# Gregor-Mendel-Institute/SNPmatch

Measured on NVIDIA B200. Metric: snp_accession_comparisons_per_sec, higher is better.
Workload: dtype f64

## Files before the change

### snpmatch_b200/csrc/api.cu

```cuda
#include "common.cuh"
#include <atomic>
#include <memory>
#include <new>
#include "pack.cuh"
#include "join.cuh"
#include "score.cuh"
#include "windows.cuh"
#include "f1.cuh"
#include "hardcall.cuh"
#include "gemm_onehot.cuh"
#include "grouped.cuh"
#include "group_sort.cuh"
#include "grouped2.cuh"
#include "pairs.cuh"
#include "pair_matrix.cuh"
#include "cross_geno.cuh"
#include <unordered_map>

namespace snpm {
thread_local std::string g_last_error;

static int grid_for(int64_t items, int threads, int n_sm, int per_sm = 16) {
    int64_t g = ceil_div64(items, threads);
    const int64_t cap = int64_t(n_sm) * per_sm;
// ... 558 lines not shown
        } else {
            SNPM_CUDA(cudaMemcpyAsync(b->d_wei.p, wei, size_t(n) * 24, cudaMemcpyHostToDevice, st));
        }
    }
    SNPM_CUDA(cudaEventRecord(b->ev_uploaded, st));
    b->ran = b->ran_windows = b->epilogue_done = false;
    return SNPM_OK;
}

static int batch_new(snpm_db *db, snpm_batch **out) {
    snpm_batch *b = new snpm_batch();
    b->db = db;
    for (int i = 0; i < SNPM_N_EVENTS; ++i) {
        if (cudaEventCreate(&b->ev[i]) != cudaSuccess) { snpm_batch_destroy(b); return fail(SNPM_E_CUDA, "cudaEventCreate failed"); }
    }
    if (cudaStreamCreateWithFlags(&b->copy_stream, cudaStreamNonBlocking) != cudaSuccess ||
        cudaEventCreateWithFlags(&b->ev_uploaded, cudaEventDisableTiming) != cudaSuccess ||
        cudaEventCreateWithFlags(&b->ev_inputs_free, cudaEventDisableTiming) != cudaSuccess ||
        cudaEventCreate(&b->ev_joined) != cudaSuccess) {
        snpm_batch_destroy(b);
        return fail(SNPM_E_CUDA, "snpm_batch_create: copy stream / events");
    }
    if (cudaMallocHost(reinterpret_cast<void **>(&b->h_status), 8 * sizeof(int)) != cudaSuccess) {
        snpm_batch_destroy(b);
        return fail(SNPM_E_NOMEM, "cudaMallocHost failed");
    }
    *out = b;
    return SNPM_OK;
}

int snpm_batch_create(snpm_db *db, int64_t n_samples, const int64_t *offsets, const int32_t *s_chrom_id, const int32_t *s_pos,
                      const double *wei, snpm_batch **out) {
    if (!db || !out) return fail(SNPM_E_ARG, "snpm_batch_create: NULL handle");
    *out = nullptr;
    SNPM_CUDA(cudaSetDevice(db->device));
    snpm_batch *b = nullptr;
    SNPM_TRY(batch_new(db, &b));
    int rc = batch_upload(b, n_samples, offsets, s_chrom_id, s_pos, wei);
    if (rc == SNPM_OK && cudaStreamSynchronize(b->copy_stream) != cudaSuccess) rc = fail(SNPM_E_CUDA, "snpm_batch_create: upload failed");
    if (rc != SNPM_OK) { snpm_batch_destroy(b); return rc; }
    *out = b;
    return SNPM_OK;
}

int snpm_batch_upload(snpm_batch *b, int64_t n_samples, const int64_t *offsets, const int32_t *s_chrom_id, const int32_t *s_pos,
                      const double *wei) {
    if (!b) return fail(SNPM_E_ARG, "snpm_batch_upload: NULL batch");
    SNPM_CUDA(cudaSetDevice(b->db->device));
    return batch_upload(b, n_samples, offsets, s_chrom_id, s_pos, wei);
}

int snpm_batch_upload_indexed(snpm_batch *b, int64_t n_samples, const int64_t *offsets, const int32_t *s_chrom_id, const int32_t *s_pos,
                              const uint16_t *wei_idx, const double *table, int32_t n_table) {
    if (!b) return fail(SNPM_E_ARG, "snpm_batch_upload_indexed: NULL batch");
    if (!wei_idx && offsets && n_samples >= 1 && offsets[n_samples] > 0) return fail(SNPM_E_ARG, "snpm_batch_upload_indexed: NULL weight indices");
    SNPM_CUDA(cudaSetDevice(b->db->device));
    return batch_upload(b, n_samples, offsets, s_chrom_id, s_pos, nullptr, wei_idx, table, n_table);
}


int snpm_group_markers(int64_t n_samples, const int64_t *offsets, const int32_t *s_chrom_id, const int32_t *s_pos, const double *wei,
                       uint8_t *out_chrom, int32_t *out_pos, uint16_t *out_gid, int64_t *out_order, double *table, int32_t table_cap,
                       int32_t *n_table) {
    if (n_samples < 1 || !offsets || !n_table || !table || table_cap < 1) return fail(SNPM_E_ARG, "snpm_group_markers: bad arguments");
    const int64_t n = offsets[n_samples];
    if (n > 0 && (!s_chrom_id || !s_pos || !wei || !out_chrom || !out_pos || !out_gid)) return fail(SNPM_E_ARG, "snpm_group_markers: NULL marker arrays");
    struct Key {
        uint64_t a, b, c;
        bool operator==(const Key &o) const { return a == o.a && b == o.b && c == o.c; }
    };
    struct KeyHash {
        size_t operator()(const Key &k) const {
            uint64_t h = k.a * 0x9E3779B97F4A7C15ull;
            h ^= (k.b + 0x7F4A7C15ull) * 0xC2B2AE3D27D4EB4Full + (h << 6) + (h >> 2);
            h ^= (k.c + 0x165667B19E3779F9ull) * 0xFF51AFD7ED558CCDull + (h << 6) + (h >> 2);
            return size_t(h ^ (h >> 29));
        }
    };
    std::unordered_map<Key, int32_t, KeyHash> ids;
    ids.reserve(4096);
    const int32_t cap = std::min<int32_t>(table_cap, 65536);
    std::vector<int32_t> gid(static_cast<size_t>(n));
    for (int64_t i = 0; i < n; ++i) {
        const double w0 = wei[3 * i], w1 = wei[3 * i + 1], w2 = wei[3 * i + 2];
        if (!(w0 >= 0.0 && w1 >= 0.0 && w2 >= 0.0) || std::isinf(w0) || std::isinf(w1) || std::isinf(w2))
            return fail(SNPM_E_ARG, "snpm_group_markers: weights must be finite and non-negative (marker %lld)", (long long)i);
        Key k;
        memcpy(&k.a, &w0, 8);
        memcpy(&k.b, &w1, 8);
        memcpy(&k.c, &w2, 8);
        if (w0 == 0.0) k.a = 0;
        if (w1 == 0.0) k.b = 0;
        if (w2 == 0.0) k.c = 0;
        auto it = ids.find(k);
        if (it == ids.end()) {
            const int32_t id = int32_t(ids.size());
            if (id >= cap) return fail(SNPM_E_RANGE, "snpm_group_markers: more than %d distinct weight triples", cap);
            table[3 * size_t(id)] = w0;
            table[3 * size_t(id) + 1] = w1;
            table[3 * size_t(id) + 2] = w2;
            it = ids.emplace(k, id).first;
        }
        gid[size_t(i)] = it->second;
        const int32_t c = s_chrom_id[i];
        if (c >= 255) return fail(SNPM_E_RANGE, "snpm_group_markers: chromosome id %d does not fit one byte", c);
    }
    const int32_t T = int32_t(ids.size());
    *n_table = T;
    {
        std::vector<int32_t> called(static_cast<size_t>(T));
        std::vector<std::vector<double>> seen(9);
        for (int32_t t = 0; t < T; ++t) {
            const double *w = table + 3 * size_t(t);
            int c = 0;
            if (w[0] == 1.0) c = 0; else if (w[2] == 1.0) c = 2; else if (w[1] == 1.0) c = 1;
            else { c = 0; if (w[2] > w[c]) c = 2; if (w[1] > w[c]) c = 1; }
            called[size_t(t)] = c;
            for (int k = 0; k < 3; ++k) seen[size_t(3 * c + k)].push_back(w[k]);
        }
        int slow[3], fast[3];
        for (int c = 0; c < 3; ++c) {
            size_t distinct[3] = {0, 0, 0};
            for (int k = 0; k < 3; ++k) {
                auto &v = seen[size_t(3 * c + k)];
                std::sort(v.begin(), v.end());
                distinct[k] = size_t(std::unique(v.begin(), v.end()) - v.begin());
            }
            const int o1 = (c + 1) % 3, o2 = (c + 2) % 3;
            if (distinct[o1] <= distinct[o2]) { slow[c] = o1; fast[c] = o2; } else { slow[c] = o2; fast[c] = o1; }
        }
        std::vector<int32_t> perm(static_cast<size_t>(T)), rank(static_cast<size_t>(T));
        for (int32_t t = 0; t < T; ++t) perm[size_t(t)] = t;
        std::sort(perm.begin(), perm.end(), [&](int32_t x, int32_t y) {
            const int cx = called[size_t(x)], cy = called[size_t(y)];
            if (cx != cy) return cx < cy;
            const double *wx_ = table + 3 * size_t(x), *wy_ = table + 3 * size_t(y);
            if (wx_[cx] != wy_[cx]) return wx_[cx] > wy_[cx];
            if (wx_[slow[cx]] != wy_[slow[cx]]) return wx_[slow[cx]] > wy_[slow[cx]];
            if (wx_[fast[cx]] != wy_[fast[cx]]) return wx_[fast[cx]] > wy_[fast[cx]];
            return x < y;
        });
        std::vector<double> sorted(static_cast<size_t>(T) * 3);
        for (int32_t r = 0; r < T; ++r) {
            rank[size_t(perm[size_t(r)])] = r;
            memcpy(&sorted[3 * size_t(r)], table + 3 * size_t(perm[size_t(r)]), 24);
        }
        memcpy(table, sorted.data(), size_t(T) * 24);
        for (int64_t i = 0; i < n; ++i) gid[size_t(i)] = rank[size_t(gid[size_t(i)])];
    }
    std::vector<int64_t> cnt(static_cast<size_t>(T) + 1);
    for (int64_t s = 0; s < n_samples; ++s) {
        const int64_t b0 = offsets[s], b1 = offsets[s + 1];
        std::fill(cnt.begin(), cnt.end(), 0);
        for (int64_t i = b0; i < b1; ++i) ++cnt[size_t(gid[size_t(i)]) + 1];
        for (int32_t t = 0; t < T; ++t) cnt[size_t(t) + 1] += cnt[size_t(t)];
        for (int64_t i = b0; i < b1; ++i) {
            const int32_t g = gid[size_t(i)];
            const int64_t o = b0 + cnt[size_t(g)]++;
            out_chrom[o] = s_chrom_id[i] < 0 ? uint8_t(255) : uint8_t(s_chrom_id[i]);
            out_pos[o] = s_pos[i];
            out_gid[o] = uint16_t(g);
            if (out_order) out_order[o] = i;
        }
    }
    return SNPM_OK;
}

static int upload_grouped(snpm_batch *b, int64_t n_samples, const int64_t *offsets, const uint8_t *chrom_u8, const int32_t *s_pos,
                          const uint32_t *packed_cp, const uint16_t *gid, const double *table, int32_t n_table,
                          const uint16_t *run_gid = nullptr, const uint32_t *run_end = nullptr, int64_t n_runs = 0) {
    if (!b) return fail(SNPM_E_ARG, "snpm_batch_upload_grouped: NULL batch");
    snpm_db *db = b->db;
    if (n_samples < 1 || !offsets || offsets[0] != 0) return fail(SNPM_E_ARG, "snpm_batch_upload_grouped: need samples and offsets starting at 0");
    for (int64_t s = 0; s < n_samples; ++s)
        if (offsets[s + 1] < offsets[s]) return fail(SNPM_E_ARG, "snpm_batch_upload_grouped: offsets must be non-decreasing");
    const int64_t n = offsets[n_samples];
    if (n >= (int64_t(1) << 31) - 2048) return fail(SNPM_E_ARG, "snpm_batch_upload_grouped: %lld markers exceed the 2^31 limit", (long long)n);
    if (n > 0 && ((!gid && !run_gid) || (!packed_cp && (!chrom_u8 || !s_pos)))) return fail(SNPM_E_ARG, "snpm_batch_upload_grouped: NULL marker arrays");
    if (run_gid && n > 0) {
        if (!run_end || n_runs < 1 || n_runs > n) return fail(SNPM_E_ARG, "snpm_batch_upload_grouped_runs: need 1..n runs");
        if (int64_t(run_end[n_runs - 1]) != n || run_end[0] == 0) return fail(SNPM_E_ARG, "snpm_batch_upload_grouped_runs: the runs must cover markers 0..n");
    }
    if (!table || n_table < 1 || n_table > 65536) return fail(SNPM_E_ARG, "snpm_batch_upload_grouped: weight table must hold 1..65536 triples");
    std::vector<double> t4(size_t(n_table) * 4);
    for (int32_t t = 0; t < n_table; ++t) {
        const double w0 = table[3 * size_t(t)], w1 = table[3 * size_t(t) + 1], w2 = table[3 * size_t(t) + 2];
        if (!(w0 >= 0.0 && w1 >= 0.0 && w2 >= 0.0) || std::isinf(w0) || std::isinf(w1) || std::isinf(w2))
            return fail(SNPM_E_ARG, "snpm_batch_upload_grouped: weights must be finite and non-negative (triple %d)", t);
        t4[4 * size_t(t)] = w0;
        t4[4 * size_t(t) + 1] = w2;
        t4[4 * size_t(t) + 2] = w1;
        t4[4 * size_t(t) + 3] = 0.0;
    }
    SNPM_CUDA(cudaSetDevice(db->device));
    b->S = n_samples;
    b->n = n;
    b->grouped = true;
    b->coded = false;
    b->pending_expand = 0;
    b->n_gtable = n_table;
    b->gchunk = b->gchunk_req;
    b->h_off.assign(offsets, offsets + n_samples + 1);
    int64_t nseg = 0;
    for (int64_t s = 0; s < n_samples; ++s) nseg += ceil_div64(offsets[s + 1] - offsets[s], b->gchunk);
    b->nseg_cap = nseg;
    SNPM_TRY(b->d_off.ensure(size_t(n_samples + 1) * 8));
    SNPM_TRY(b->d_chrom8.ensure(size_t(n)));
    SNPM_TRY(b->d_chrom.ensure(size_t(n) * 4));
    SNPM_TRY(b->d_pos.ensure(size_t(n) * 4));
    SNPM_TRY(b->d_gid.ensure(size_t(n) * 2));
    SNPM_TRY(b->d_gtable.ensure(size_t(n_table) * 32));
    cudaStream_t st = b->copy_stream;
    SNPM_CUDA(cudaStreamWaitEvent(st, b->ev_inputs_free, 0));
    SNPM_CUDA(cudaMemcpyAsync(b->d_off.p, offsets, size_t(n_samples + 1) * 8, cudaMemcpyHostToDevice, st));
    b->h_gtable.assign(t4.begin(), t4.end());
    SNPM_CUDA(cudaMemcpyAsync(b->d_gtable.p, b->h_gtable.data(), size_t(n_table) * 32, cudaMemcpyHostToDevice, st));
    if (n) {
        if (run_gid) {
            const size_t bad_off = (size_t(n_runs) * 6 + 15) & ~size_t(15);
            SNPM_TRY(b->d_runs.ensure(bad_off + 16));
            uint32_t *d_end = b->d_runs.as<uint32_t>();
            uint16_t *d_rg = reinterpret_cast<uint16_t *>(d_end + n_runs);
            b->d_runs_bad = reinterpret_cast<int *>(static_cast<char *>(b->d_runs.p) + bad_off);
            SNPM_CUDA(cudaMemsetAsync(b->d_runs_bad, 0, sizeof(int), st));
            SNPM_CUDA(cudaMemcpyAsync(d_end, run_end, size_t(n_runs) * 4, cudaMemcpyHostToDevice, st));
            SNPM_CUDA(cudaMemcpyAsync(d_rg, run_gid, size_t(n_runs) * 2, cudaMemcpyHostToDevice, st));
            b->pending_expand |= 1;
            b->pending_runs = n_runs;
        } else {
            b->d_runs_bad = nullptr;
            SNPM_CUDA(cudaMemcpyAsync(b->d_gid.p, gid, size_t(n) * 2, cudaMemcpyHostToDevice, st));
        }
        if (packed_cp) {
            SNPM_TRY(b->d_wei_idx.ensure(size_t(n) * 4));
            SNPM_CUDA(cudaMemcpyAsync(b->d_wei_idx.p, packed_cp, size_t(n) * 4, cudaMemcpyHostToDevice, st));
            b->pending_expand |= 2;
        } else {
            SNPM_CUDA(cudaMemcpyAsync(b->d_chrom8.p, chrom_u8, size_t(n), cudaMemcpyHostToDevice, st));
            SNPM_CUDA(cudaMemcpyAsync(b->d_pos.p, s_pos, size_t(n) * 4, cudaMemcpyHostToDevice, st));
            b->pending_expand |= 4;
        }
    }
    SNPM_CUDA(cudaEventRecord(b->ev_uploaded, st));
    b->ran = b->ran_windows = b->epilogue_done = false;
    return SNPM_OK;
}

int snpm_batch_upload_grouped(snpm_batch *b, int64_t n_samples, const int64_t *offsets, const uint8_t *chrom_u8, const int32_t *s_pos,
                              const uint16_t *gid, const double *table, int32_t n_table) {
    return upload_grouped(b, n_samples, offsets, chrom_u8, s_pos, nullptr, gid, table, n_table);
}

int snpm_batch_upload_grouped_packed(snpm_batch *b, int64_t n_samples, const int64_t *offsets, const uint32_t *chrom_pos, const uint16_t *gid,
                                     const double *table, int32_t n_table) {
    return upload_grouped(b, n_samples, offsets, nullptr, nullptr, chrom_pos, gid, table, n_table);
}

int snpm_batch_upload_grouped_runs(snpm_batch *b, int64_t n_samples, const int64_t *offsets, const uint32_t *chrom_pos, const uint16_t *run_gid,
                                   const uint32_t *run_end, int64_t n_runs, const double *table, int32_t n_table) {
    return upload_grouped(b, n_samples, offsets, nullptr, nullptr, chrom_pos, nullptr, table, n_table, run_gid, run_end, n_runs);
}

static int upload_coded(snpm_batch *b, int64_t n_samples, const int64_t *offsets, const uint32_t *chrom_pos, const uint16_t *codes,
                        const uint32_t *codes32, const double *wtable, int32_t n_wtable) {
    if (!b) return fail(SNPM_E_ARG, "snpm_batch_upload_coded: NULL batch");
    if (codes32 && n_wtable > 1024) return fail(SNPM_E_ARG, "snpm_batch_upload_coded32: three codes share one word only up to 1024 weight values (%d given)", n_wtable);
    snpm_db *db = b->db;
    if (n_samples < 1 || !offsets || offsets[0] != 0) return fail(SNPM_E_ARG, "snpm_batch_upload_coded: need samples and offsets starting at 0");
    for (int64_t s = 0; s < n_samples; ++s)
        if (offsets[s + 1] < offsets[s]) return fail(SNPM_E_ARG, "snpm_batch_upload_coded: offsets must be non-decreasing");
    const int64_t n = offsets[n_samples];
    if (n >= (int64_t(1) << 31) - 2048) return fail(SNPM_E_ARG, "snpm_batch_upload_coded: %lld markers exceed the 2^31 limit", (long long)n);
    if (n > 0 && (!chrom_pos || (!codes && !codes32))) return fail(SNPM_E_ARG, "snpm_batch_upload_coded: NULL marker arrays");
    if (!wtable || n_wtable < 1 || n_wtable > 65536) return fail(SNPM_E_ARG, "snpm_batch_upload_coded: the weight table must hold 1..65536 values");
    for (int32_t t = 0; t < n_wtable; ++t)
        if (!(wtable[t] >= 0.0) || std::isinf(wtable[t])) return fail(SNPM_E_ARG, "snpm_batch_upload_coded: weights must be finite and non-negative (entry %d)", t);
    if (!b->gchunk_set) b->gchunk_req = db->stride > G2_WX ? G2_MAX_CHUNK : 320;
    if (b->gchunk_req % GR_BLOCK || b->gchunk_req > G2_MAX_CHUNK)
        return fail(SNPM_E_ARG, "snpm_batch_upload_coded: the group chunk must be a multiple of %d and at most %d rows (it is %d)", GR_BLOCK, G2_MAX_CHUNK, b->gchunk_req);
    SNPM_CUDA(cudaSetDevice(db->device));
    b->S = n_samples;
    b->n = n;
    b->grouped = true;
    b->coded = true;
    b->codes_packed = codes32 != nullptr;
    b->pending_expand = 2;
    b->d_runs_bad = nullptr;
    b->n_wtable = n_wtable;
    int bits = 1;
    while ((1 << bits) < n_wtable) ++bits;
    b->code_bits = bits;
    b->key_bits = 3 * bits + 2;
    b->gchunk = b->gchunk_req;
    b->h_off.assign(offsets, offsets + n_samples + 1);
    int64_t nseg = 0;
    std::vector<int32_t> tile_first(size_t(n_samples) + 1), tile_sample;
    for (int64_t s = 0; s < n_samples; ++s) {
        const int64_t ns = offsets[s + 1] - offsets[s];
        nseg += ceil_div64(ns, b->gchunk);
        tile_first[size_t(s)] = int32_t(tile_sample.size());
        for (int64_t t = 0; t < ceil_div64(ns, RS_TILE); ++t) tile_sample.push_back(int32_t(s));
    }
    tile_first[size_t(n_samples)] = int32_t(tile_sample.size());
    b->nseg_cap = nseg;
    b->n_sort_tiles = int64_t(tile_sample.size());
    const size_t key_bytes = b->key_bits <= 32 ? 4 : 8;
    SNPM_TRY(b->d_off.ensure(size_t(n_samples + 1) * 8));
    SNPM_TRY(b->d_chrom.ensure(size_t(n) * 4));
    SNPM_TRY(b->d_pos.ensure(size_t(n) * 4));
    SNPM_TRY(b->d_wei_idx.ensure(size_t(n) * 4));
    SNPM_TRY(b->d_codes.ensure(size_t(n) * 6));
    SNPM_TRY(b->d_wtable.ensure(size_t(n_wtable) * 8));
    SNPM_TRY(b->d_key_a.ensure(size_t(n) * key_bytes));
    SNPM_TRY(b->d_pair_db_tmp.ensure(size_t(n) * 4));
    SNPM_TRY(b->d_pair_s_tmp.ensure(size_t(n) * 4));
    SNPM_TRY(b->d_tile_sample.ensure(std::max<size_t>(tile_sample.size(), 1) * 4));
    SNPM_TRY(b->d_tile_first.ensure(size_t(n_samples + 1) * 4));
    SNPM_TRY(b->d_tile_hist.ensure(std::max<size_t>(tile_sample.size(), 1) * (size_t(GH_MAX_GROUPS) * 4 + 8)));
    SNPM_TRY(b->d_blk_chg.ensure(size_t(std::max<int64_t>(nseg, 1)) * (size_t(b->gchunk / GR_BLOCK) * 8 + 12) + size_t(SO_BUCKETS) * 4 + 16));
    SNPM_TRY(b->d_seg_order.ensure(size_t(std::max<int64_t>(nseg, 1)) * 16));
    SNPM_TRY(b->d_work_counter.ensure(256));
    SNPM_TRY(b->d_hash.ensure(size_t(n_samples) * GH_SLOTS * 8));
    SNPM_TRY(b->d_slot_gid.ensure(size_t(n_samples) * GH_SLOTS * 2));
    SNPM_TRY(b->d_ngroups.ensure(size_t(n_samples) * 4));
    SNPM_TRY(b->d_group_overflow.ensure(size_t(n_samples) * 4));
    SNPM_TRY(b->d_gkeys.ensure(size_t(n_samples) * GH_MAX_GROUPS * key_bytes));
    SNPM_TRY(b->d_gw.ensure(size_t(n_samples) * GH_MAX_GROUPS * 32));
    SNPM_TRY(b->d_goff.ensure(size_t(n_samples) * (GH_MAX_GROUPS + 1) * 4));
    SNPM_TRY(b->d_gid.ensure(size_t(n) * 2));
    cudaStream_t st = b->copy_stream;
    SNPM_CUDA(cudaStreamWaitEvent(st, b->ev_inputs_free, 0));
    b->h_gtable.assign(wtable, wtable + n_wtable);
    b->h_tiles.assign(tile_first.begin(), tile_first.end());
    b->h_tiles.insert(b->h_tiles.end(), tile_sample.begin(), tile_sample.end());
    SNPM_CUDA(cudaMemcpyAsync(b->d_off.p, offsets, size_t(n_samples + 1) * 8, cudaMemcpyHostToDevice, st));
    SNPM_CUDA(cudaMemcpyAsync(b->d_wtable.p, b->h_gtable.data(), size_t(n_wtable) * 8, cudaMemcpyHostToDevice, st));
    SNPM_CUDA(cudaMemcpyAsync(b->d_tile_first.p, b->h_tiles.data(), size_t(n_samples + 1) * 4, cudaMemcpyHostToDevice, st));
    if (!tile_sample.empty())
        SNPM_CUDA(cudaMemcpyAsync(b->d_tile_sample.p, b->h_tiles.data() + n_samples + 1, tile_sample.size() * 4, cudaMemcpyHostToDevice, st));
    if (n) {
        SNPM_CUDA(cudaMemcpyAsync(b->d_wei_idx.p, chrom_pos, size_t(n) * 4, cudaMemcpyHostToDevice, st));
        if (codes32) SNPM_CUDA(cudaMemcpyAsync(b->d_codes.p, codes32, size_t(n) * 4, cudaMemcpyHostToDevice, st));
        else SNPM_CUDA(cudaMemcpyAsync(b->d_codes.p, codes, size_t(n) * 6, cudaMemcpyHostToDevice, st));
    }
    SNPM_CUDA(cudaEventRecord(b->ev_uploaded, st));
    b->ran = b->ran_windows = b->epilogue_done = false;
    return SNPM_OK;
}

int snpm_batch_upload_coded(snpm_batch *b, int64_t n_samples, const int64_t *offsets, const uint32_t *chrom_pos, const uint16_t *codes,
                            const double *wtable, int32_t n_wtable) {
    return upload_coded(b, n_samples, offsets, chrom_pos, codes, nullptr, wtable, n_wtable);
}

int snpm_batch_upload_coded32(snpm_batch *b, int64_t n_samples, const int64_t *offsets, const uint32_t *chrom_pos, const uint32_t *codes32,
                              const double *wtable, int32_t n_wtable) {
    return upload_coded(b, n_samples, offsets, chrom_pos, nullptr, codes32, wtable, n_wtable);
}

int snpm_batch_coded_timings(snpm_batch *b, float *ms, int n) {
    if (!b || !ms || n < 4) return fail(SNPM_E_ARG, "snpm_batch_coded_timings: need room for 4 floats");
    if (!b->coded || !b->ran) return fail(SNPM_E_STATE, "snpm_batch_coded_timings: run a coded batch first");
    SNPM_CUDA(cudaSetDevice(b->db->device));
    SNPM_CUDA(cudaStreamSynchronize(b->db->stream));
    for (int i = 0; i < n; ++i) ms[i] = 0.f;
    cudaEventElapsedTime(&ms[0], b->ev[SNPM_EV_START], b->ev_joined);
    cudaEventElapsedTime(&ms[1], b->ev_joined, b->ev[SNPM_EV_JOIN]);
    cudaEventElapsedTime(&ms[2], b->ev[SNPM_EV_JOIN], b->ev[SNPM_EV_SCORE]);
    cudaEventElapsedTime(&ms[3], b->ev[SNPM_EV_SCORE], b->ev[SNPM_EV_COMBINE]);
    return SNPM_OK;
}

int snpm_pack_markers(int64_t n, const uint8_t *chrom_u8, const int32_t *pos, uint32_t *out) {
    if (n < 0 || (n > 0 && (!chrom_u8 || !pos || !out))) return fail(SNPM_E_ARG, "snpm_pack_markers: bad arguments");
    for (int64_t i = 0; i < n; ++i) {
        const uint32_t c = chrom_u8[i] == 255 ? 31u : uint32_t(chrom_u8[i]);
        if ((chrom_u8[i] != 255 && c > 30u) || pos[i] < 0 || pos[i] >= (1 << 27))
            return fail(SNPM_E_RANGE, "snpm_pack_markers: marker %lld (chromosome id %u, position %d) does not fit 5 + 27 bits", (long long)i, c, pos[i]);
        out[i] = (c << 27) | uint32_t(pos[i]);
    }
    return SNPM_OK;
}

int snpm_pack_coded(int64_t n, const int32_t *chrom_id, const int32_t *pos, const uint16_t *codes, uint32_t *chrom_pos, uint32_t *codes32) {
    if (n < 0 || (n > 0 && (!chrom_id || !pos || !chrom_pos || (codes32 && !codes)))) return fail(SNPM_E_ARG, "snpm_pack_coded: bad arguments");
    uint32_t bad = 0u;
    for (int64_t i = 0; i < n; ++i) {
        const int32_t c = chrom_id[i], p = pos[i];
        bad |= uint32_t(c > 30) | uint32_t(p < 0) | uint32_t(p >= (1 << 27));
        chrom_pos[i] = ((c < 0 ? 31u : uint32_t(c)) << 27) | (uint32_t(p) & ((1u << 27) - 1u));
    }
    if (codes32)
        for (int64_t i = 0; i < n; ++i) {
            const uint32_t a = codes[3 * i], h = codes[3 * i + 1], t = codes[3 * i + 2];
            bad |= uint32_t((a | h | t) > 1023u);
            codes32[i] = a | (h << 10) | (t << 20);
        }
    if (bad) return fail(SNPM_E_RANGE, "snpm_pack_coded: a chromosome id above 30, a position outside 27 bits or a code above 1023");
    return SNPM_OK;
}

int snpm_batch_guard_counts(snpm_batch *b, int32_t *counts) {
    if (!b || !counts) return fail(SNPM_E_ARG, "snpm_batch_guard_counts: NULL argument");
    if (!b->grouped) { for (int64_t s = 0; s < b->rangen(); ++s) counts[s] = 0; return SNPM_OK; }
    if (!b->epilogue_done) return fail(SNPM_E_STATE, "snpm_batch_guard_counts: run the epilogue first");
    if (b->rangen() == 0) return SNPM_OK;
    SNPM_CUDA(cudaSetDevice(b->db->device));
    SNPM_CUDA(cudaMemcpyAsync(counts, b->d_guard.as<int32_t>() + b->range0(), size_t(b->rangen()) * 4, cudaMemcpyDeviceToHost, b->db->stream));
    SNPM_CUDA(cudaStreamSynchronize(b->db->stream));
    return SNPM_OK;
}

int snpm_batch_set_result_range(snpm_batch *b, int64_t first_sample, int64_t n_samples) {
    if (!b || first_sample < 0 || n_samples < -1) return fail(SNPM_E_ARG, "snpm_batch_set_result_range: bad range");
    b->res0 = first_sample;
    b->resn = n_samples;
    return SNPM_OK;
}

int snpm_batch_set_track_pairs(snpm_batch *b, int on) {
    if (!b) return fail(SNPM_E_ARG, "snpm_batch_set_track_pairs: NULL batch");
    b->track_pairs = on != 0;
    return SNPM_OK;
}

int snpm_batch_set_chunk_rows(snpm_batch *b, int32_t rows) {
    if (!b || rows < 1 || rows > 1000000) return fail(SNPM_E_ARG, "snpm_batch_set_chunk_rows: 1..1000000 rows");
    b->chunk_rows_req = rows;
    return SNPM_OK;
}

int snpm_batch_set_group_chunk(snpm_batch *b, int32_t rows) {
    if (!b || rows < 16 || rows > GR_MAX_CHUNK || rows % 8) return fail(SNPM_E_ARG, "snpm_batch_set_group_chunk: 16..%d rows, a multiple of 8", GR_MAX_CHUNK);
    b->gchunk_req = rows;
    b->gchunk_set = true;
    return SNPM_OK;
}

static void ipc_close_peers(snpm_batch *b);

int snpm_batch_destroy(snpm_batch *b) {
    if (!b) return SNPM_OK;
    cudaSetDevice(b->db->device);
    cudaStreamSynchronize(b->db->stream);
    if (b->copy_stream) { cudaStreamSynchronize(b->copy_stream); cudaStreamDestroy(b->copy_stream); }
    if (b->ev_uploaded) cudaEventDestroy(b->ev_uploaded);
    if (b->ev_inputs_free) cudaEventDestroy(b->ev_inputs_free);
    if (b->ev_joined) cudaEventDestroy(b->ev_joined);
    if (b->ev_fork) cudaEventDestroy(b->ev_fork);
    if (b->ev_join) cudaEventDestroy(b->ev_join);
    DevBuf *bufs[] = {&b->d_off, &b->d_chrom, &b->d_pos, &b->d_wei, &b->d_filter, &b->d_match_row, &b->d_tile_cnt, &b->d_tile_off,
                      &b->d_prefix, &b->d_pair_db, &b->d_pair_s, &b->d_pair_w, &b->d_mstart, &b->d_seg_off, &b->d_part_score,
                      &b->d_part_ninfo, &b->d_red, &b->d_matches, &b->d_ninfo64, &b->d_prob, &b->d_L, &b->d_LR, &b->d_status,
                      &b->d_win_count, &b->d_win_off, &b->d_win_begin, &b->d_win_end, &b->d_kmax, &b->d_win_L, &b->d_win_LR,
                      &b->d_win_ident, &b->d_win_amb, &b->d_win_row_off, &b->d_row_acc, &b->d_row_score, &b->d_row_ninfo, &b->d_row_L, &b->d_row_ident, &b->d_f1_acc, &b->d_f1_part, &b->d_f1_out, &b->d_pair_code, &b->d_wei_idx, &b->d_wei_table,
                      &b->d_chrom8, &b->d_gid, &b->d_gtable, &b->d_pair_gid, &b->d_part_int, &b->d_guard, &b->d_runs,
                      &b->d_codes, &b->d_wtable, &b->d_key_a, &b->d_key_b, &b->d_idx_a, &b->d_idx_b, &b->d_pair_db_tmp, &b->d_pair_s_tmp,
                      &b->d_tile_sample, &b->d_tile_first, &b->d_tile_hist, &b->d_blk_chg, &b->d_seg_order, &b->d_work_counter, &b->d_hash, &b->d_slot_gid, &b->d_ngroups,
                      &b->d_group_overflow, &b->d_gkeys, &b->d_gw, &b->d_goff, &b->d_segsel, &b->d_segsel_off, &b->d_flags, &b->d_flag_counts};
    for (DevBuf *d : bufs) d->release();
    for (int i = 0; i < SNPM_N_EVENTS; ++i)
        if (b->ev[i]) cudaEventDestroy(b->ev[i]);
    if (b->h_status) cudaFreeHost(b->h_status);
    if (b->h_tail) cudaFreeHost(b->h_tail);
    if (b->ev_fetched) cudaEventDestroy(b->ev_fetched);
    if (b->ev_results) cudaEventDestroy(b->ev_results);
    ipc_close_peers(b);
    delete b;
    return SNPM_OK;
}

int snpm_batch_set_row_filter(snpm_batch *b, const int64_t *sorted_rows, int64_t n) {
    if (!b || n < 0) return fail(SNPM_E_ARG, "snpm_batch_set_row_filter: bad arguments");
    for (int64_t i = 1; i < n; ++i)
        if (sorted_rows[i] <= sorted_rows[i - 1]) return fail(SNPM_E_ARG, "snpm_batch_set_row_filter: rows must be strictly ascending");
    SNPM_CUDA(cudaSetDevice(b->db->device));
    b->has_filter = sorted_rows != nullptr;
    b->n_filter = b->has_filter ? n : 0;
    SNPM_TRY(b->d_filter.ensure(size_t(std::max<int64_t>(n, 1)) * 8));
    if (b->has_filter && n) {
        SNPM_CUDA(cudaMemcpyAsync(b->d_filter.p, sorted_rows, size_t(n) * 8, cudaMemcpyHostToDevice, b->db->stream));
        SNPM_CUDA(cudaStreamSynchronize(b->db->stream));
    }
    return SNPM_OK;
}

int snpm_batch_set_segregation_filter(snpm_batch *b, const uint32_t *sel, int64_t S, int32_t words) {
    if (!b) return fail(SNPM_E_ARG, "snpm_batch_set_segregation_filter: NULL batch");
    if (!sel) {
        b->has_seg = false;
        b->seg_S = 0;
        return SNPM_OK;
    }
    snpm_db *db = b->db;
    if (S < 1 || words != db->stride)
        return fail(SNPM_E_ARG, "snpm_batch_set_segregation_filter: need S >= 1 selections of snpm_db_row_words() = %d words (got S = %lld, %d words)",
                    db->stride, (long long)S, words);
    std::vector<int32_t> off(size_t(S) + 1, 0);
    std::vector<uint32_t> pairs;
    for (int64_t s = 0; s < S; ++s) {
        for (int32_t w = 0; w < words; ++w) {
            const uint32_t m = sel[size_t(s) * words + w];
            const int64_t first = int64_t(w) * 32;
            const uint32_t valid = first >= db->n_acc ? 0u : (db->n_acc - first >= 32 ? 0xffffffffu : (1u << (db->n_acc - first)) - 1u);
            if (m & ~valid) return fail(SNPM_E_ARG, "snpm_batch_set_segregation_filter: sample %lld selects accessions beyond the panel's %d", (long long)s, db->n_acc);
            if (m) {
                pairs.push_back(uint32_t(w));
                pairs.push_back(m);
            }
        }
        if (pairs.size() / 2 > size_t(INT32_MAX)) return fail(SNPM_E_ARG, "snpm_batch_set_segregation_filter: selections too large");
        off[size_t(s) + 1] = int32_t(pairs.size() / 2);
    }
    SNPM_CUDA(cudaSetDevice(db->device));
    SNPM_TRY(b->d_segsel.ensure(std::max<size_t>(pairs.size(), 2) * 4));
    SNPM_TRY(b->d_segsel_off.ensure(off.size() * 4));
    if (!pairs.empty()) SNPM_CUDA(cudaMemcpyAsync(b->d_segsel.p, pairs.data(), pairs.size() * 4, cudaMemcpyHostToDevice, db->stream));
    SNPM_CUDA(cudaMemcpyAsync(b->d_segsel_off.p, off.data(), off.size() * 4, cudaMemcpyHostToDevice, db->stream));
    SNPM_CUDA(cudaStreamSynchronize(db->stream));
    b->has_seg = true;
    b->seg_S = S;
    return SNPM_OK;
}

int snpm_batch_count_flagged_pairs(snpm_batch *b, const uint8_t *flags, int64_t *counts) {
    if (!b || !counts || (b->n > 0 && !flags)) return fail(SNPM_E_ARG, "snpm_batch_count_flagged_pairs: bad arguments");
    if (!b->ran) return fail(SNPM_E_STATE, "snpm_batch_count_flagged_pairs: run the batch first");
    snpm_db *db = b->db;
    SNPM_CUDA(cudaSetDevice(db->device));
    cudaStream_t st = db->stream;
    SNPM_TRY(b->d_flag_counts.ensure(size_t(b->S) * 8));
    SNPM_CUDA(cudaMemsetAsync(b->d_flag_counts.p, 0, size_t(b->S) * 8, st));
    if (b->n > 0) {
        SNPM_TRY(b->d_flags.ensure(size_t(b->n)));
        SNPM_CUDA(cudaMemcpyAsync(b->d_flags.p, flags, size_t(b->n), cudaMemcpyHostToDevice, st));
        k_count_flagged_pairs<<<int(ceil_div64(b->n, 256)), 256, 0, st>>>(b->d_match_row.as<int32_t>(), b->d_flags.as<uint8_t>(), b->n,
                                                                          b->d_off.as<int64_t>(), b->S, b->d_flag_counts.as<unsigned long long>());
        SNPM_KERNEL_CHECK();
    }
    SNPM_CUDA(cudaMemcpyAsync(counts, b->d_flag_counts.p, size_t(b->S) * 8, cudaMemcpyDeviceToHost, st));
    SNPM_CUDA(cudaStreamSynchronize(st));
    return SNPM_OK;
}

static int batch_join(snpm_batch *b, int algo) {
    snpm_db *db = b->db;
    cudaStream_t st = db->stream;
    const int64_t n = b->n, S = b->S;
    const int64_t n_tiles = ceil_div64(n, JOIN_TILE);
    SNPM_TRY(b->d_match_row.ensure(size_t(n) * 4));
    SNPM_TRY(b->d_tile_cnt.ensure(size_t(n_tiles) * 4));
    SNPM_TRY(b->d_tile_off.ensure(size_t(n_tiles) * 4));
    SNPM_TRY(b->d_prefix.ensure(size_t(n + 1) * 4));
    SNPM_TRY(b->d_pair_db.ensure(size_t(n) * 4));
    SNPM_TRY(b->d_pair_s.ensure(size_t(n) * 4));
    if (b->coded) {  }
    else if (b->grouped) SNPM_TRY(b->d_pair_gid.ensure(size_t(n) * 2 + 16));
    else SNPM_TRY(b->d_pair_w.ensure(size_t(n) * 32));
    SNPM_TRY(b->d_mstart.ensure(size_t(S + 1) * 4));
    SNPM_TRY(b->d_seg_off.ensure(size_t(S + 1) * 4));
    SNPM_TRY(b->d_status.ensure(8 * sizeof(int)));
    SNPM_CUDA(cudaStreamWaitEvent(st, b->ev_uploaded, 0));
    SNPM_CUDA(cudaMemsetAsync(b->d_status.p, 0, 8 * sizeof(int), st));
    if (b->grouped && b->pending_expand && n > 0) {
        if (b->pending_expand & 1) {
            const uint32_t *d_end = b->d_runs.as<uint32_t>();
            k_expand_runs<<<int(ceil_div64(b->pending_runs * 32, 256)), 256, 0, st>>>(d_end, reinterpret_cast<const uint16_t *>(d_end + b->pending_runs),
                                                                                 int32_t(b->pending_runs), n, b->d_gid.as<uint16_t>(), b->d_runs_bad);
        }
        if (b->pending_expand & 4) k_expand_chrom<<<int(ceil_div64(n, 256)), 256, 0, st>>>(b->d_chrom8.as<uint8_t>(), n, b->d_chrom.as<int32_t>());
        SNPM_KERNEL_CHECK();
        b->pending_expand &= 2;
    }
    if (b->grouped && b->d_runs_bad) SNPM_CUDA(cudaMemcpyAsync(b->d_status.as<int>() + 4, b->d_runs_bad, sizeof(int), cudaMemcpyDeviceToDevice, st));
    if (!b->peer_red.empty() && b->ipc_step > 0 && b->d_red.p == b->ipc_ptr) {
        k_wait_peers_done<<<1, 32, 0, st>>>(reinterpret_cast<const uint32_t *>(static_cast<const char *>(b->d_red.p) + b->ipc_flags_off),
                                            int32_t(b->peer_red.size()), b->ipc_step, b->d_status.as<int>());
        SNPM_KERNEL_CHECK();
    }
    if (algo == 0) algo = (n / S) * 8 >= db->n_rows ? 2 : 1;
    if (b->grouped) algo = 1;
    const int64_t *filter = b->has_filter ? b->d_filter.as<int64_t>() : nullptr;
    if (b->coded && S > 0) SNPM_CUDA(cudaMemsetAsync(b->d_group_overflow.p, 0, size_t(S) * 4, st));
    if (n_tiles > 0) {
        if (algo == 2)
            k_join_mergepath<<<int(n_tiles), 256, 0, st>>>(b->d_chrom.as<int32_t>(), b->d_pos.as<int32_t>(), n, b->d_off.as<int64_t>(), S,
                                                         db->d_pos, db->d_chr_regions, db->n_chr, filter, b->n_filter, db->row0_global,
                                                         b->d_match_row.as<int32_t>(), b->d_tile_cnt.as<int32_t>(), b->d_status.as<int>());
        else
            k_join_search<<<int(n_tiles), JOIN_TILE, 0, st>>>(b->d_chrom.as<int32_t>(), b->d_pos.as<int32_t>(), n, b->d_off.as<int64_t>(), S,
                                                            db->d_pos, db->d_chr_regions, db->n_chr, db->d_bucket, db->d_bucket_off, db->bucket_shift,
                                                            filter, b->n_filter, db->row0_global,
                                                            b->d_match_row.as<int32_t>(), b->d_tile_cnt.as<int32_t>(), b->d_status.as<int>(), (b->grouped && !b->coded) ? 0 : 1,
                                                            db->d_bitmap, db->d_bm_first_row, db->d_bm_off,
                                                            (b->grouped && (b->pending_expand & 2)) ? b->d_wei_idx.as<uint32_t>() : nullptr);
        SNPM_KERNEL_CHECK();
        if (b->has_seg) {
            static_assert(SEGP_THREADS == JOIN_TILE, "the segregation filter recounts the join's tiles");
            k_segregating_pairs<<<int(n_tiles), SEGP_THREADS, 0, st>>>(db->d_packed, db->stride, b->d_off.as<int64_t>(), S, n, b->d_segsel.as<uint2>(),
                                                                      b->d_segsel_off.as<int32_t>(), b->d_match_row.as<int32_t>(), b->d_tile_cnt.as<int32_t>());
            SNPM_KERNEL_CHECK();
            b->launches += 1;
        }
        k_scan_tiles<<<1, 1024, 0, st>>>(b->d_tile_cnt.as<int32_t>(), n_tiles, b->d_tile_off.as<int32_t>(), b->d_prefix.as<int32_t>() + n);
        SNPM_KERNEL_CHECK();
        if (b->coded) {
            unsigned long long *hash = b->d_hash.as<unsigned long long>();
            SNPM_CUDA(cudaMemsetAsync(hash, 0, size_t(S) * GH_SLOTS * 8, st));
            if (b->key_bits <= 32)
                k_scatter_pairs_coded<uint32_t><<<int(n_tiles), SC_THREADS, 0, st>>>(b->d_match_row.as<int32_t>(), n, b->d_tile_off.as<int32_t>(), b->d_codes.as<uint16_t>(),
                        b->d_wtable.as<double>(), b->n_wtable, b->code_bits, b->d_prefix.as<int32_t>(), b->d_pair_db_tmp.as<int32_t>(), b->d_pair_s_tmp.as<int32_t>(),
                        b->d_key_a.as<uint32_t>(), b->d_status.as<int>(), b->d_off.as<int64_t>(), S, hash, b->d_group_overflow.as<int>(),
                        b->codes_packed ? b->d_codes.as<uint32_t>() : nullptr);
            else
                k_scatter_pairs_coded<uint64_t><<<int(n_tiles), SC_THREADS, 0, st>>>(b->d_match_row.as<int32_t>(), n, b->d_tile_off.as<int32_t>(), b->d_codes.as<uint16_t>(),
                        b->d_wtable.as<double>(), b->n_wtable, b->code_bits, b->d_prefix.as<int32_t>(), b->d_pair_db_tmp.as<int32_t>(), b->d_pair_s_tmp.as<int32_t>(),
                        b->d_key_a.as<uint64_t>(), b->d_status.as<int>(), b->d_off.as<int64_t>(), S, hash, b->d_group_overflow.as<int>(),
                        b->codes_packed ? b->d_codes.as<uint32_t>() : nullptr);
        } else if (b->grouped)
            k_scatter_pairs_grouped<<<int(n_tiles), JOIN_TILE, 0, st>>>(b->d_match_row.as<int32_t>(), n, b->d_tile_off.as<int32_t>(),
                                                                      b->d_gid.as<uint16_t>(), b->n_gtable, b->d_prefix.as<int32_t>(), b->d_pair_db.as<int32_t>(),
                                                                      b->d_pair_s.as<int32_t>(), b->d_pair_gid.as<uint16_t>(), b->d_status.as<int>());
        else
            k_scatter_pairs<<<int(n_tiles), JOIN_TILE, 0, st>>>(b->d_match_row.as<int32_t>(), n, b->d_tile_off.as<int32_t>(), b->d_wei.as<double>(),
                                                              b->d_prefix.as<int32_t>(), b->d_pair_db.as<int32_t>(), b->d_pair_s.as<int32_t>(),
                                                              b->d_pair_w.as<double>());
        SNPM_KERNEL_CHECK();
        b->launches += 3;
    } else {
        SNPM_CUDA(cudaMemsetAsync(b->d_prefix.p, 0, 4, st));
    }
    k_sample_ranges<<<1, 1024, 0, st>>>(b->d_prefix.as<int32_t>(), b->d_off.as<int64_t>(), S, b->grouped ? b->gchunk : b->chunk_rows, b->d_mstart.as<int32_t>(),
                                        b->d_seg_off.as<int32_t>());
    SNPM_KERNEL_CHECK();
    b->launches += 1;
    return SNPM_OK;
}

}

template <typename KeyT>
static int batch_group_sort_t(snpm_batch *b) {
    snpm_db *db = b->db;
    cudaStream_t st = db->stream;
    const int tiles = int(b->n_sort_tiles);
    if (tiles == 0 || b->n == 0) return SNPM_OK;
    const int32_t *mstart = b->d_mstart.as<int32_t>(), *tsample = b->d_tile_sample.as<int32_t>(), *tfirst = b->d_tile_first.as<int32_t>();
    uint32_t *hist = b->d_tile_hist.as<uint32_t>();
    int2 *range = reinterpret_cast<int2 *>(hist + (size_t(tiles) << 11));
    SNPM_CUDA(smem_attr<k_group_place>(64 * 1024));
    KeyT *gkeys = b->d_gkeys.as<KeyT>();
    k_group_rank<KeyT><<<int(b->S), 1024, 0, st>>>(b->d_hash.as<unsigned long long>(), b->d_wtable.as<double>(), b->code_bits, b->d_slot_gid.as<uint16_t>(),
                                                   b->d_ngroups.as<int32_t>(), gkeys, b->d_gw.as<double4>(), b->d_group_overflow.as<int>());
    int64_t n_max = 0, jcap1 = 1;
    for (int64_t s = 0; s < b->S; ++s) {
        n_max = std::max(n_max, b->h_off[size_t(s) + 1] - b->h_off[size_t(s)]);
        jcap1 = std::max(jcap1, ceil_div64(b->h_off[size_t(s) + 1] - b->h_off[size_t(s)], b->gchunk));
    }
    const char *force = getenv("SNPM_GROUP_KERNEL");
    const bool fits = n_max <= GP_MAX_PAIRS;
    const bool want = force ? !strcmp(force, "sample") : (n_max <= 32768 || b->S >= 128);
    if (fits && want) {
        SNPM_CUDA(smem_attr<k_group_sample<KeyT>>(int(GP_SMEM)));
        const size_t ncap = size_t(std::max<int64_t>(b->nseg_cap, 1));
        int32_t *cost = reinterpret_cast<int32_t *>(b->d_blk_chg.as<unsigned long long>() + ncap * size_t(b->gchunk / GR_BLOCK));
        int32_t *buckets = cost + ncap;
        const size_t zbytes = ncap * (size_t(b->gchunk / GR_BLOCK) * 8 + 4) + size_t(SO_BUCKETS) * 4;
        int2 *br = reinterpret_cast<int2 *>(reinterpret_cast<unsigned char *>(b->d_blk_chg.p) + ((zbytes + 7) & ~size_t(7)));
        SNPM_CUDA(cudaMemsetAsync(b->d_blk_chg.p, 0, zbytes, st));
        k_group_sample<KeyT><<<int(b->S), 32 * GP_WARPS, GP_SMEM, st>>>(
            b->d_key_a.as<KeyT>(), b->d_hash.as<unsigned long long>(), b->d_slot_gid.as<uint16_t>(), b->d_ngroups.as<int32_t>(), b->d_gid.as<uint16_t>(),
            b->d_pair_db_tmp.as<int32_t>(), b->d_pair_s_tmp.as<int32_t>(), b->d_pair_db.as<int32_t>(), b->track_pairs ? b->d_pair_s.as<int32_t>() : nullptr,
            b->d_goff.as<int32_t>(), gkeys, mstart, b->d_seg_off.as<int32_t>(), b->gchunk, b->code_bits, b->d_blk_chg.as<unsigned long long>(), cost,
            int32_t(jcap1), buckets, br, b->d_work_counter.as<unsigned int>());
        k_order_place<<<int(b->S), 256, 0, st>>>(buckets, br, b->d_seg_off.as<int32_t>(), mstart, b->gchunk, b->d_seg_order.as<int4>());
        SNPM_KERNEL_CHECK();
        b->launches += 3;
        return SNPM_OK;
    }
    k_tile_ranges<<<(tiles + 255) / 256, 256, 0, st>>>(mstart, tsample, tfirst, tiles, range);
    k_group_ids<KeyT><<<tiles, RS_THREADS, 0, st>>>(b->d_key_a.as<KeyT>(), range, tsample, b->d_hash.as<unsigned long long>(), b->d_slot_gid.as<uint16_t>(),
                                                    b->d_ngroups.as<int32_t>(), b->d_gid.as<uint16_t>(), hist);
    k_group_scan<<<int(b->S), 1024, 0, st>>>(hist, tfirst, b->d_ngroups.as<int32_t>(), b->d_goff.as<int32_t>());
    const size_t nseg_cap = size_t(std::max<int64_t>(b->nseg_cap, 1));
    int32_t *seg_cost = reinterpret_cast<int32_t *>(b->d_blk_chg.as<unsigned long long>() + nseg_cap * size_t(b->gchunk / GR_BLOCK));
    int32_t *bucket_cnt = seg_cost + nseg_cap;
    const size_t zero_bytes = nseg_cap * (size_t(b->gchunk / GR_BLOCK) * 8 + 4) + size_t(SO_BUCKETS) * 4;
    int2 *seg_br = reinterpret_cast<int2 *>(reinterpret_cast<unsigned char *>(b->d_blk_chg.p) + ((zero_bytes + 7) & ~size_t(7)));
    int64_t jcap = 1;
    for (int64_t s = 0; s < b->S; ++s) jcap = std::max(jcap, ceil_div64(b->h_off[size_t(s) + 1] - b->h_off[size_t(s)], b->gchunk));
    cudaStream_t aux = b->copy_stream;
    if (!b->ev_fork) SNPM_CUDA(cudaEventCreateWithFlags(&b->ev_fork, cudaEventDisableTiming));
    if (!b->ev_join) SNPM_CUDA(cudaEventCreateWithFlags(&b->ev_join, cudaEventDisableTiming));
    SNPM_CUDA(cudaEventRecord(b->ev_fork, st));
    SNPM_CUDA(cudaStreamWaitEvent(aux, b->ev_fork, 0));
    SNPM_CUDA(cudaMemsetAsync(b->d_blk_chg.p, 0, zero_bytes, aux));
    k_group_marks<KeyT><<<int(b->S), 1024, 0, aux>>>(b->d_goff.as<int32_t>(), gkeys, b->d_ngroups.as<int32_t>(), mstart, b->d_seg_off.as<int32_t>(), b->gchunk,
                                                     b->code_bits, b->d_blk_chg.as<unsigned long long>(), seg_cost, int32_t(jcap), bucket_cnt, seg_br);
    k_order_place<<<int(b->S), 256, 0, aux>>>(bucket_cnt, seg_br, b->d_seg_off.as<int32_t>(), mstart, b->gchunk, b->d_seg_order.as<int4>());
    SNPM_CUDA(cudaEventRecord(b->ev_join, aux));
    k_group_place<<<tiles, RS_THREADS, size_t(GH_MAX_GROUPS) * 20, st>>>(b->d_gid.as<uint16_t>(), b->d_pair_db_tmp.as<int32_t>(), b->d_pair_s_tmp.as<int32_t>(),
                                                                        b->d_pair_db.as<int32_t>(), b->track_pairs ? b->d_pair_s.as<int32_t>() : nullptr, mstart, tsample,
                                                                        tfirst, range, hist, b->d_ngroups.as<int32_t>(), b->d_goff.as<int32_t>(), b->d_work_counter.as<unsigned int>());
    SNPM_CUDA(cudaStreamWaitEvent(st, b->ev_join, 0));
    SNPM_KERNEL_CHECK();
    b->launches += 7;
    return SNPM_OK;
}

static int launch_grouped2(snpm_batch *b, bool skip_db_hets) {
    snpm_db *db = b->db;
    cudaStream_t st = db->stream;
    Group2Args g = {};
    g.packed = db->d_packed; g.stride = db->stride; g.pair_db = b->d_pair_db.as<int32_t>();
    g.blk_chg = b->d_blk_chg.as<unsigned long long>(); g.gw = b->d_gw.as<double>();
    g.seg_off = b->d_seg_off.as<int32_t>(); g.mstart = b->d_mstart.as<int32_t>(); g.S = int32_t(b->S); g.chunk = b->gchunk;
    g.part_score = b->d_part_score.as<double>(); g.part_int = b->d_part_int.as<int32_t>(); g.a_pad = db->stride * 32;
    if (db->stride <= G2_WX) { g.n_slices = 1; g.wx = (db->stride + 1) & ~1; }
    else { g.wx = 32; g.n_slices = (db->stride + 31) / 32; }
    g.teams = std::min(G2_THREADS / g.wx, G2_MAX_TEAMS);
    g.order = b->d_seg_order.as<int4>();
    g.work_counter = b->d_work_counter.as<unsigned int>();
    const int64_t n_items = std::max<int64_t>(b->nseg_cap, 1) * g.n_slices;
    if (n_items >= (int64_t(1) << 31) - (int64_t(1) << 20)) return fail(SNPM_E_ARG, "snpm_batch_run: %lld work items exceed the 2^31 limit", (long long)n_items);
    constexpr int ring = 64;
    const size_t smem = size_t(g.teams) * g2_team_smem(g.wx, g.chunk, ring);
    if (smem > 226 * 1024) return fail(SNPM_E_ARG, "snpm_batch_run: group chunk %d needs %zu bytes of shared memory", g.chunk, smem);
    const int grid = int(std::min<int64_t>(db->n_sm, ceil_div64(n_items, g.teams)));
#define G2_LAUNCH(SK, WXV)                                                                                                        \
    do {                                                                                                                          \
        SNPM_CUDA((smem_attr<k_score_grouped2<SK, WXV, ring>>(226 * 1024)));                                                    \
        k_score_grouped2<SK, WXV, ring><<<grid, G2_THREADS, smem, st>>>(g);                                                       \
    } while (0)
    if (g.wx == G2_WX) {
        if (skip_db_hets) G2_LAUNCH(true, G2_WX); else G2_LAUNCH(false, G2_WX);
    } else if (g.wx == 32) {
        if (skip_db_hets) G2_LAUNCH(true, 32); else G2_LAUNCH(false, 32);
    } else {
        if (skip_db_hets) G2_LAUNCH(true, 0); else G2_LAUNCH(false, 0);
    }
#undef G2_LAUNCH
    SNPM_KERNEL_CHECK();
    b->launches += 1;
    return SNPM_OK;
}

extern "C" {

static int batch_alloc_outputs(snpm_batch *b, int64_t nseg) {
    snpm_db *db = b->db;
    const int64_t a_pad = int64_t(db->stride) * 32;
    const int64_t SA = b->S * int64_t(db->n_acc);
    SNPM_TRY(b->d_part_score.ensure(size_t(std::max<int64_t>(nseg, 1)) * a_pad * 8));
    SNPM_TRY(b->d_part_ninfo.ensure(size_t(std::max<int64_t>(nseg, 1)) * a_pad * 4));
    SNPM_TRY(b->d_red.ensure(size_t(b->S) * size_t(b->red_pitch()) * 8));
    if (b->grouped) SNPM_TRY(b->d_part_int.ensure(size_t(std::max<int64_t>(nseg, 1)) * a_pad * 4));
    SNPM_TRY(b->d_matches.ensure(size_t(SA) * 8));
    SNPM_TRY(b->d_ninfo64.ensure(size_t(SA) * 8));
    SNPM_TRY(b->d_prob.ensure(size_t(SA) * 8));
    SNPM_TRY(b->d_L.ensure(size_t(SA) * 8));
    SNPM_TRY(b->d_LR.ensure(size_t(SA) * 8));
    return SNPM_OK;
}

static void rec(snpm_batch *b, int which) {
    cudaEventRecord(b->ev[which], b->db->stream);
    b->ev_rec[which] = true;
}

int snpm_batch_run(snpm_batch *b, int skip_db_hets, int mode) {
    if (!b) return fail(SNPM_E_ARG, "snpm_batch_run: NULL batch");
    snpm_db *db = b->db;
    SNPM_CUDA(cudaSetDevice(db->device));
    cudaStream_t st = db->stream;
    const int kernel_mode = mode & 0xff, algo = (mode >> 8) & 0xff;
    if (kernel_mode < 0 || kernel_mode > 2) return fail(SNPM_E_ARG, "snpm_batch_run: unknown kernel mode %d", kernel_mode);
    if ((kernel_mode == 2) != b->grouped)
        return fail(SNPM_E_STATE, "snpm_batch_run: kernel mode 2 scores batches uploaded with snpm_batch_upload_grouped, and only those");
    if (algo > 2) return fail(SNPM_E_ARG, "snpm_batch_run: unknown join algorithm %d", algo);
    if (b->has_seg && kernel_mode == 2)
        return fail(SNPM_E_STATE, "snpm_batch_run: the segregation filter is honoured by kernel modes 0 and 1 only; clear it first");
    if (b->has_seg && b->seg_S != b->S)
        return fail(SNPM_E_ARG, "snpm_batch_run: the segregation filter holds %lld selections for %lld samples", (long long)b->seg_S, (long long)b->S);
    b->launches = 0;
    for (int i = 0; i < SNPM_N_EVENTS; ++i) b->ev_rec[i] = false;
    SNPM_TRY(batch_alloc_outputs(b, b->nseg_cap));
    rec(b, SNPM_EV_START);
    SNPM_TRY(batch_join(b, algo));
    rec(b, SNPM_EV_JOIN);
    ScoreArgs a = {};
    a.packed = db->d_packed;
    a.stride = db->stride;
    a.pair_db = b->d_pair_db.as<int32_t>();
    a.pair_w = b->d_pair_w.as<double>();
    a.seg_off = b->d_seg_off.as<int32_t>();
    a.mstart = b->d_mstart.as<int32_t>();
    a.S = int32_t(b->S);
    a.chunk = b->chunk_rows;
    a.table = 0;
    a.part_score = b->d_part_score.as<double>();
    a.part_ninfo = b->d_part_ninfo.as<int32_t>();
    a.a_pad = db->stride * 32;
    if (kernel_mode == 2 && b->coded) {
        cudaEventRecord(b->ev_joined, st);
        if (b->key_bits <= 32) SNPM_TRY(batch_group_sort_t<uint32_t>(b)); else SNPM_TRY(batch_group_sort_t<uint64_t>(b));
        rec(b, SNPM_EV_JOIN);
        if (b->nseg_cap > 0 && b->n > 0) {
            SNPM_TRY(launch_grouped2(b, skip_db_hets != 0));
        }
        rec(b, SNPM_EV_SCORE);
        dim3 cgrid((a.a_pad + 31) / 32, unsigned(b->S));
        k_combine_grouped<<<cgrid, 32 * CG_PARTS, 0, st>>>(a.part_score, b->d_part_int.as<int32_t>(), a.a_pad, db->stride, db->n_acc, a.seg_off, a.mstart,
                                                 b->d_group_overflow.as<int>(), b->d_red.as<double>());
        SNPM_KERNEL_CHECK();
        b->launches += 1;
        rec(b, SNPM_EV_COMBINE);
        SNPM_CUDA(cudaEventRecord(b->ev_inputs_free, st));
        b->ran = true;
        b->ran_windows = false;
        b->epilogue_done = false;
        return SNPM_OK;
    }
    if (kernel_mode == 2) {
        if (b->nseg_cap > 0) {
            GroupArgs g = {};
            g.packed = db->d_packed; g.stride = db->stride; g.pair_db = a.pair_db; g.pair_gid = b->d_pair_gid.as<uint16_t>();
            g.table = b->d_gtable.as<double>(); g.seg_off = a.seg_off; g.mstart = a.mstart; g.S = a.S; g.chunk = b->gchunk;
            g.part_score = a.part_score; g.part_int = b->d_part_int.as<int32_t>(); g.a_pad = a.a_pad;
            const int nsl = (db->stride + GR_MAX_WX - 1) / GR_MAX_WX;
            g.wx = ((db->stride + nsl - 1) / nsl + 1) & ~1;
            g.spc = std::min(GR_THREADS / g.wx, GR_MAX_TEAMS);
            const size_t gsmem = size_t(g.spc) * grouped_team_smem(g.wx, g.chunk);
            int64_t jmax = 0;
            for (int64_t smp = 0; smp < b->S; ++smp)
                jmax = std::max(jmax, ceil_div64(b->h_off[size_t(smp) + 1] - b->h_off[size_t(smp)], b->gchunk));
            g.jmax = int32_t(jmax);
            dim3 ggrid(unsigned(ceil_div64(b->S * jmax, g.spc)), unsigned((db->stride + g.wx - 1) / g.wx));
#define GR_LAUNCH(SK, WXV)                                                     \
    do {                                                                       \
        SNPM_CUDA((smem_attr<k_score_grouped<SK, WXV>>(220 * 1024)));          \
        k_score_grouped<SK, WXV><<<ggrid, GR_THREADS, gsmem, st>>>(g);         \
    } while (0)
            if (g.wx == GR_MAX_WX) {
                if (skip_db_hets) GR_LAUNCH(true, GR_MAX_WX); else GR_LAUNCH(false, GR_MAX_WX);
            } else {
                if (skip_db_hets) GR_LAUNCH(true, 0); else GR_LAUNCH(false, 0);
            }
#undef GR_LAUNCH
            SNPM_KERNEL_CHECK();
            b->launches += 1;
        }
        rec(b, SNPM_EV_SCORE);
        dim3 cgrid((a.a_pad + 31) / 32, unsigned(b->S));
        k_combine_grouped<<<cgrid, 32 * CG_PARTS, 0, st>>>(a.part_score, b->d_part_int.as<int32_t>(), a.a_pad, db->stride, db->n_acc, a.seg_off, a.mstart,
                                                 nullptr, b->d_red.as<double>());
        SNPM_KERNEL_CHECK();
        b->launches += 1;
        rec(b, SNPM_EV_COMBINE);
        SNPM_CUDA(cudaEventRecord(b->ev_inputs_free, st));
        b->ran = true;
        b->ran_windows = false;
        b->epilogue_done = false;
        return SNPM_OK;
    }
    if (kernel_mode == 1 && b->chunk_rows != SNPM_CHUNK_ROWS)
        return fail(SNPM_E_STATE, "snpm_batch_run: the popcount kernel works in %d-row chunks (its sums are exact in any chunking); set the chunk back", SNPM_CHUNK_ROWS);
    if (kernel_mode == 1 && b->nseg_cap > 0) {
        SNPM_TRY(b->d_pair_code.ensure(size_t(std::max<int64_t>(b->n, 1))));
        k_pair_codes<<<int(ceil_div64(b->n, 256)), 256, 0, st>>>(a.pair_w, b->d_prefix.as<int32_t>() + b->n, b->d_pair_code.as<uint8_t>());
        SNPM_KERNEL_CHECK();
        HardArgs h = {};
        h.packed = a.packed; h.stride = a.stride; h.pair_db = a.pair_db; h.pair_code = b->d_pair_code.as<uint8_t>();
        h.seg_off = a.seg_off; h.mstart = a.mstart; h.S = a.S; h.chunk = a.chunk;
        h.part_score = a.part_score; h.part_ninfo = a.part_ninfo; h.a_pad = a.a_pad; h.status = b->d_status.as<int>();
        const int wx = std::min<int>(db->stride, HC_THREADS), spc = std::min(HC_THREADS / wx, HC_MAX_SEGS);
        h.wx = wx;
        h.spc = spc;
        dim3 hgrid(unsigned(ceil_div64(b->nseg_cap, spc)), unsigned((db->stride + wx - 1) / wx));
        const size_t hsmem = size_t(spc) * SNPM_CHUNK_ROWS * 5;
        if (skip_db_hets) {
            SNPM_CUDA(smem_attr<k_score_hard<true>>(64 * 1024));
            k_score_hard<true><<<hgrid, HC_THREADS, hsmem, st>>>(h);
        } else {
            SNPM_CUDA(smem_attr<k_score_hard<false>>(64 * 1024));
            k_score_hard<false><<<hgrid, HC_THREADS, hsmem, st>>>(h);
        }
        SNPM_KERNEL_CHECK();
        b->launches += 2;
    } else {
        SNPM_TRY(launch_score(st, a, int(b->nseg_cap), skip_db_hets != 0));
        if (b->nseg_cap > 0) b->launches += 1;
    }
    rec(b, SNPM_EV_SCORE);
    dim3 cgrid((db->n_acc + 31) / 32, unsigned(b->S));
    k_combine<<<cgrid, 32, 0, st>>>(a.part_score, a.part_ninfo, a.a_pad, db->n_acc, a.seg_off, a.mstart, 0, nullptr, nullptr, b->d_red.as<double>());
    SNPM_KERNEL_CHECK();
    b->launches += 1;
    rec(b, SNPM_EV_COMBINE);
    SNPM_CUDA(cudaEventRecord(b->ev_inputs_free, st));
    b->ran = true;
    b->ran_windows = false;
    b->epilogue_done = false;
    return SNPM_OK;
}

int snpm_batch_epilogue(snpm_batch *b) {
    if (!b) return fail(SNPM_E_ARG, "snpm_batch_epilogue: NULL batch");
    if (!b->ran) return fail(SNPM_E_STATE, "snpm_batch_epilogue: run the batch first");
    if (b->grouped && b->epilogue_done) return fail(SNPM_E_STATE, "snpm_batch_epilogue: the epilogue of a grouped batch runs once per run");
    snpm_db *db = b->db;
    SNPM_CUDA(cudaSetDevice(db->device));
    const int64_t r0 = b->range0(), rn = b->rangen();
    if (r0 < 0 || rn < 0 || r0 + rn > b->S) return fail(SNPM_E_ARG, "snpm_batch_epilogue: result range [%lld, %lld) outside the %lld samples", (long long)r0, (long long)(r0 + rn), (long long)b->S);
    rec(b, SNPM_EV_EPI_START);
    const int64_t pitch = b->red_pitch(), A = db->n_acc;
    if (rn > 0) {
        if (b->grouped) {
            SNPM_TRY(b->d_guard.ensure(size_t(b->S) * 4));
            SNPM_CUDA(cudaMemsetAsync(b->d_guard.as<int32_t>() + r0, 0, size_t(rn) * 4, db->stream));
            dim3 fgrid((db->n_acc + 255) / 256, unsigned(rn));
            k_grouped_finalize<<<fgrid, 256, 0, db->stream>>>(b->d_red.as<double>() + r0 * pitch, db->n_acc, b->d_guard.as<int32_t>() + r0);
            SNPM_KERNEL_CHECK();
            b->launches += 1;
        }
        SNPM_CUDA(launch_epilogue(db->stream, rn, b->d_red.as<double>() + r0 * pitch, pitch, db->n_acc, 1, 0, 0.0,
                                  b->d_matches.as<int64_t>() + r0 * A, b->d_ninfo64.as<int64_t>() + r0 * A,
                                  b->d_prob.as<double>() + r0 * A, b->d_L.as<double>() + r0 * A, b->d_LR.as<double>() + r0 * A));
    }
    SNPM_KERNEL_CHECK();
    b->launches += 1;
    rec(b, SNPM_EV_EPI_END);
    b->epilogue_done = true;
    return SNPM_OK;
}

int snpm_batch_wait(snpm_batch *b, float *ms_device) {
    if (!b) return fail(SNPM_E_ARG, "snpm_batch_wait: NULL batch");
    snpm_db *db = b->db;
    SNPM_CUDA(cudaSetDevice(db->device));
    if (b->d_status.p) SNPM_CUDA(cudaMemcpyAsync(b->h_status, b->d_status.p, 8 * sizeof(int), cudaMemcpyDeviceToHost, db->stream));
    else memset(b->h_status, 0, 8 * sizeof(int));
    SNPM_CUDA(cudaStreamSynchronize(db->stream));
    if (ms_device) {
        *ms_device = 0.f;
        if (b->ev_rec[SNPM_EV_START] && b->ev_rec[SNPM_EV_COMBINE]) {
            float t = 0.f;
            cudaEventElapsedTime(&t, b->ev[SNPM_EV_START], b->ev[SNPM_EV_COMBINE]);
            *ms_device += t;
        }
        if (b->ev_rec[SNPM_EV_EPI_START] && b->ev_rec[SNPM_EV_EPI_END]) {
            float t = 0.f;
            cudaEventElapsedTime(&t, b->ev[SNPM_EV_EPI_START], b->ev[SNPM_EV_EPI_END]);
            *ms_device += t;
        }
    }
    if (b->h_status[0] > 0)
        return fail(SNPM_E_ARG, "sample markers are not sorted by (database chromosome order, position) or repeat a position (%d places)", b->h_status[0]);
    if (b->h_status[1] > 0)
        return fail(SNPM_E_ASSERT, "provided y is greater than n (%d window cells; likeliTest, snpmatch.py:43)", b->h_status[1]);
    if (b->h_status[2] > 0)
        return fail(SNPM_E_ARG, "identity table too short for %d window cells", b->h_status[2]);
    if (b->h_status[3] > 0)
        return fail(SNPM_E_ARG, "kernel mode 1 needs one-hot weights (called genotypes); %d matched markers are not", b->h_status[3]);
    if (b->h_status[4] > 0)
        return fail(SNPM_E_ARG, "%d matched markers carry a weight-triple id outside the table (or run-length coded ids do not ascend)", b->h_status[4]);
    if (b->h_status[5] > 0)
        return fail(SNPM_E_STATE, "peer reduce: a rank did not arrive within thirty seconds (every rank must run and reduce the same batches in the same order)");
    return SNPM_OK;
}

int snpm_batch_timings(snpm_batch *b, float *ms, int n) {
    if (!b || !ms || n < 6) return fail(SNPM_E_ARG, "snpm_batch_timings: need room for 6 floats");
    SNPM_CUDA(cudaSetDevice(b->db->device));
    SNPM_CUDA(cudaStreamSynchronize(b->db->stream));
    for (int i = 0; i < n; ++i) ms[i] = 0.f;
    auto el = [&](int a, int c) {
        float t = 0.f;
        if (b->ev_rec[a] && b->ev_rec[c]) cudaEventElapsedTime(&t, b->ev[a], b->ev[c]);
        return t;
    };
    ms[0] = el(SNPM_EV_START, SNPM_EV_JOIN);
    ms[1] = el(SNPM_EV_JOIN, SNPM_EV_SCORE);
    ms[2] = el(SNPM_EV_SCORE, SNPM_EV_COMBINE);
    ms[3] = el(SNPM_EV_EPI_START, SNPM_EV_EPI_END);
    ms[4] = el(SNPM_EV_START, SNPM_EV_COMBINE) + ms[3];
// ... 891 lines not shown
```

### snpmatch_b200/csrc/common.cuh

```cuda
#pragma once
#include <cuda_runtime.h>
#include <stdint.h>
#include <stdarg.h>
#include <stdio.h>
#include <stdlib.h>
#include <string.h>
#include <string>
#include <vector>
#include <algorithm>
#include <cmath>

#include "../../include/snpmatch_b200.h"

namespace snpm {

extern thread_local std::string g_last_error;

inline int fail(int code, const char *fmt, ...) __attribute__((format(printf, 2, 3)));
inline int fail(int code, const char *fmt, ...) {
    char buf[512];
    va_list ap;
    va_start(ap, fmt);
    vsnprintf(buf, sizeof(buf), fmt, ap);
    va_end(ap);
    g_last_error = buf;
    return code;
}

#define SNPM_CUDA(call)                                                                          \
    do {                                                                                         \
        cudaError_t e__ = (call);                                                                \
        if (e__ != cudaSuccess)                                                                  \
            return snpm::fail(SNPM_E_CUDA, "%s:%d %s -> %s", __FILE__, __LINE__, #call,          \
                              cudaGetErrorString(e__));                                          \
    } while (0)

#define SNPM_TRY(call)                 \
    do {                               \
        int rc__ = (call);             \
        if (rc__ != SNPM_OK) return rc__; \
    } while (0)

static inline bool snpm_sync_debug() {
    static int v = -1;
    if (v < 0) v = getenv("SNPM_SYNC_DEBUG") ? 1 : 0;
    return v == 1;
}
#define SNPM_KERNEL_CHECK()                                              \
    do {                                                                 \
        SNPM_CUDA(cudaGetLastError());                                   \
        if (snpm_sync_debug()) SNPM_CUDA(cudaDeviceSynchronize());       \
    } while (0)

struct DevBuf {
    void *p = nullptr;
    size_t cap = 0;
    int ensure(size_t bytes) {
        if (bytes <= cap && p) return SNPM_OK;
        if (p) { cudaFree(p); p = nullptr; cap = 0; }
        size_t want = bytes < 256 ? 256 : bytes;
        cudaError_t e = cudaMalloc(&p, want);
        if (e != cudaSuccess) {
            p = nullptr;
            return fail(SNPM_E_NOMEM, "cudaMalloc(%zu bytes) failed: %s", want, cudaGetErrorString(e));
        }
        cap = want;
        return SNPM_OK;
    }
    void release() {
        if (p) cudaFree(p);
        p = nullptr;
        cap = 0;
    }
    template <typename T> T *as() const { return reinterpret_cast<T *>(p); }
};

static inline int64_t ceil_div64(int64_t a, int64_t b) { return (a + b - 1) / b; }

}

struct snpm_db {
    int device = 0;
    int64_t n_rows = 0;
    int32_t n_acc = 0;
    int32_t n_words = 0;
    int32_t stride = 0;
    int64_t row0_global = 0;
    int32_t n_chr = 0;
    int n_sm = 148;
    uint64_t *d_packed = nullptr;
    int32_t *d_pos = nullptr;
    int64_t *d_chr_regions = nullptr;
    int32_t *d_bucket = nullptr;
    int32_t *d_bucket_off = nullptr;
    int bucket_shift = 0;
    unsigned long long *d_bitmap = nullptr;
    int32_t *d_bm_first_row = nullptr;
    int64_t *d_bm_off = nullptr;
    std::vector<int64_t> h_chr_regions;
    cudaStream_t stream = nullptr;
    bool own_stream = false;
    snpm::DevBuf scratch;
    struct snpm_batch *scratch_batch_ = nullptr;
};

enum { SNPM_EV_START = 0, SNPM_EV_JOIN, SNPM_EV_SCORE, SNPM_EV_COMBINE, SNPM_EV_EPI_START, SNPM_EV_EPI_END, SNPM_EV_RED_START, SNPM_EV_RED_END, SNPM_N_EVENTS };

struct snpm_batch {
    snpm_db *db = nullptr;
    int64_t S = 0;
    int64_t n = 0;
    int64_t nseg_cap = 0;
    std::vector<int64_t> h_off;
    snpm::DevBuf d_off, d_chrom, d_pos, d_wei, d_filter;
    int64_t n_filter = 0;
    bool has_filter = false;
    snpm::DevBuf d_segsel, d_segsel_off;
    int64_t seg_S = 0;
    bool has_seg = false;
    snpm::DevBuf d_flags, d_flag_counts;
    snpm::DevBuf d_match_row, d_tile_cnt, d_tile_off, d_prefix, d_pair_db, d_pair_s, d_pair_w;
    snpm::DevBuf d_mstart, d_seg_off;
    snpm::DevBuf d_part_score, d_part_ninfo, d_red, d_matches, d_ninfo64, d_prob, d_L, d_LR, d_status;
    int32_t n_windows = 0;
    int64_t bin_len = 0;
    double lr_thres = 3.841;
    snpm::DevBuf d_win_count, d_win_off, d_win_begin, d_win_end, d_kmax, d_win_L, d_win_LR, d_win_ident, d_win_amb;
    snpm::DevBuf d_win_nrows, d_win_zero, d_win_red;
    int64_t kmax_len = 0;
    bool win_pending = false;
    bool win_reduced = false;
    snpm::DevBuf d_win_row_off, d_row_acc, d_row_score, d_row_ninfo, d_row_L, d_row_ident;
    snpm::DevBuf d_f1_acc, d_f1_part, d_f1_out;
    snpm::DevBuf d_pair_code;
    snpm::DevBuf d_wei_idx, d_wei_table;
    bool grouped = false;
    int32_t n_gtable = 0;
    int32_t chunk_rows = SNPM_CHUNK_ROWS, chunk_rows_req = SNPM_CHUNK_ROWS;
    int32_t gchunk = 320;
    int32_t gchunk_req = 320;
    bool gchunk_set = false;
    bool coded = false;
    bool codes_packed = false;
    int32_t n_wtable = 0, code_bits = 0, key_bits = 0;
    int64_t n_sort_tiles = 0;
    snpm::DevBuf d_codes, d_wtable, d_key_a, d_key_b, d_idx_a, d_idx_b, d_pair_db_tmp, d_pair_s_tmp, d_tile_sample, d_tile_first,
                 d_tile_hist, d_blk_chg, d_seg_order, d_work_counter, d_hash, d_slot_gid, d_ngroups, d_group_overflow, d_gkeys, d_gw, d_goff;
    bool track_pairs = true;
    cudaEvent_t ev_fork = nullptr, ev_join = nullptr;
    cudaEvent_t ev_joined = nullptr;
    snpm::DevBuf d_chrom8, d_gid, d_gtable, d_pair_gid, d_part_int, d_guard, d_runs;
    std::vector<double> h_gtable;
    std::vector<int32_t> h_tiles;
    int pending_expand = 0;
    int64_t pending_runs = 0;
    int *d_runs_bad = nullptr;
    int64_t red_pitch() const { return (grouped ? 3 : 2) * int64_t(db->n_acc) + 2; }
    bool ran = false, ran_windows = false, epilogue_done = false;
    int launches = 0;
    cudaStream_t copy_stream = nullptr;
    cudaEvent_t ev_uploaded = nullptr, ev_inputs_free = nullptr;
    cudaEvent_t ev[SNPM_N_EVENTS] = {};
    bool ev_rec[SNPM_N_EVENTS] = {};
    int *h_status = nullptr;
    cudaEvent_t ev_fetched = nullptr, ev_results = nullptr;
    double *h_tail = nullptr;
    int64_t h_tail_cap = 0;
    int64_t *pend_m = nullptr;
    bool fetch_pending = false;
    int64_t res0 = 0, resn = -1;
    void *ipc_ptr = nullptr;
    std::vector<void *> peer_red;
    int32_t ipc_rank = -1;
    size_t ipc_flags_off = 0;
    uint32_t ipc_step = 0;
    int64_t range0() const { return resn < 0 ? 0 : res0; }
    int64_t rangen() const { return resn < 0 ? S : resn; }
};
```

### snpmatch_b200/csrc/group_sort.cuh

```cuda
#pragma once
#include "common.cuh"
#include "join.cuh"

namespace snpm {

constexpr int RS_THREADS = 256;
constexpr int RS_PER_THREAD = 8;
constexpr int RS_TILE = RS_THREADS * RS_PER_THREAD;

__host__ __device__ __forceinline__ int gs_slow_class(int c) { return c == 2 ? 0 : 2; }
__host__ __device__ __forceinline__ int gs_fast_class(int c) { return c == 1 ? 0 : 1; }
__host__ __device__ __forceinline__ int gs_field_shift(int c, int which, int b) {
    return which == c ? 2 * b : (which == gs_slow_class(c) ? b : 0);
}
template <typename KeyT>
__host__ __device__ __forceinline__ uint32_t gs_code(KeyT key, int which, int b) {
    const int c = int(key >> (3 * b)) & 3;
    return uint32_t(key >> gs_field_shift(c, which, b)) & ((1u << b) - 1u);
}

constexpr int GH_SLOTS = 4096;
constexpr int GH_MAX_GROUPS = 2048;

__device__ __forceinline__ uint32_t gh_hash(unsigned long long key) { return uint32_t((key * 0x9E3779B97F4A7C15ull) >> 52); }
__device__ __forceinline__ void gh_insert(unsigned long long *__restrict__ table, unsigned long long key, int *overflow) {
    const unsigned long long want = key + 1ull;
    uint32_t h = gh_hash(key);
    for (int probe = 0; probe < GH_SLOTS; ++probe) {
        unsigned long long cur = __ldcg(table + h);
        if (cur == 0ull) cur = atomicCAS(table + h, 0ull, want);
        if (cur == 0ull || cur == want) return;
        h = (h + 1u) & uint32_t(GH_SLOTS - 1);
    }
    atomicExch(overflow, 1);
}
__device__ __forceinline__ uint32_t gh_find(const unsigned long long *__restrict__ table, unsigned long long key) {
    const unsigned long long want = key + 1ull;
    uint32_t h = gh_hash(key);
    for (int probe = 0; probe < GH_SLOTS; ++probe) {
        const unsigned long long cur = __ldg(table + h);
        if (cur == want || cur == 0ull) break;
        h = (h + 1u) & uint32_t(GH_SLOTS - 1);
    }
    return h;
}

constexpr int SC_THREADS = 256;
constexpr int SC_PER = JOIN_TILE / SC_THREADS;
constexpr int SC_SLOTS = 1024;
template <typename KeyT>
__global__ void __launch_bounds__(SC_THREADS) k_scatter_pairs_coded(
        const int32_t *__restrict__ match_row, int64_t n, const int32_t *__restrict__ tile_off, const uint16_t *__restrict__ codes,
        const double *__restrict__ wtable, int32_t n_table, int32_t code_bits, int32_t *__restrict__ prefix,
        int32_t *__restrict__ pair_db, int32_t *__restrict__ pair_s, KeyT *__restrict__ key, int *status,
        const int64_t *__restrict__ off, int64_t S, unsigned long long *__restrict__ hash, int *__restrict__ overflow,
        const uint32_t *__restrict__ codes32) {
    constexpr int NW = SC_THREADS / 32;
    __shared__ int s_cnt[SC_PER][NW];
    __shared__ int64_t s_first_sm, s_first_end;
    __shared__ unsigned long long s_seen[SC_SLOTS];
    const int lane = threadIdx.x & 31, warp = threadIdx.x >> 5;
    const int64_t i0 = int64_t(blockIdx.x) * JOIN_TILE;
    int32_t row[SC_PER];
    uint32_t cw[SC_PER];
#pragma unroll
    for (int j = 0; j < SC_PER; ++j) {
        const int64_t i = i0 + j * SC_THREADS + threadIdx.x;
        row[j] = i < n ? match_row[i] : -1;
    }
#pragma unroll
    for (int j = 0; j < SC_PER; ++j) {
        const int64_t i = i0 + j * SC_THREADS + threadIdx.x;
        cw[j] = (codes32 != nullptr && i < n) ? codes32[i] : 0u;
    }
    const int32_t base0 = tile_off[blockIdx.x];
#pragma unroll
    for (int j = 0; j < SC_SLOTS / SC_THREADS; ++j) s_seen[j * SC_THREADS + threadIdx.x] = 0ull;
    uint32_t bal[SC_PER];
#pragma unroll
    for (int j = 0; j < SC_PER; ++j) {
        bal[j] = __ballot_sync(0xffffffffu, row[j] >= 0);
        if (lane == 0) s_cnt[j][warp] = __popc(bal[j]);
    }
    if (threadIdx.x == 0) {
        int64_t lo = 0, hi = S;
        while (hi - lo > 1) {
            const int64_t mid = (lo + hi) >> 1;
            if (off[mid] <= i0) lo = mid; else hi = mid;
        }
        s_first_sm = lo;
        s_first_end = off[lo + 1];
    }
    __syncthreads();
    const int64_t s_first = s_first_sm, first_end = s_first_end;
    int32_t base = base0;
#pragma unroll
    for (int j = 0; j < SC_PER; ++j) {
        const int64_t i = i0 + j * SC_THREADS + threadIdx.x;
        int before = 0, total = 0;
#pragma unroll
        for (int w = 0; w < NW; ++w) {
            const int c = s_cnt[j][w];
            before += w < warp ? c : 0;
            total += c;
        }
        const int32_t p = base + before + __popc(bal[j] & ((1u << lane) - 1u));
        base += total;
        unsigned long long ins = ~0ull, fold = 0ull;
        bool solo = false;
        int64_t smp = 0;
        if (i < n) {
            prefix[i] = p;
            if (row[j] >= 0) {
                pair_db[p] = row[j];
                pair_s[p] = int32_t(i);
                uint32_t cd[3];
                if (codes32 != nullptr) {
                    const uint32_t v = cw[j];
                    cd[0] = v & 1023u; cd[2] = (v >> 10) & 1023u; cd[1] = (v >> 20) & 1023u;
                } else {
                    cd[0] = codes[3 * i]; cd[2] = codes[3 * i + 1]; cd[1] = codes[3 * i + 2];
                }
                bool bad = false;
#pragma unroll
                for (int k = 0; k < 3; ++k)
                    if (int32_t(cd[k]) >= n_table) { bad = true; cd[k] = 0; }
                if (bad) atomicAdd(status + 4, 1);
                const double w0 = __ldg(wtable + cd[0]), w1 = __ldg(wtable + cd[1]), w2 = __ldg(wtable + cd[2]);
                int c;
                if (w0 == 1.0) c = 0; else if (w1 == 1.0) c = 1; else if (w2 == 1.0) c = 2;
                else { c = 0; if (w1 > w0) c = 1; if (w2 > (c ? w1 : w0)) c = 2; }
                const int b = code_bits;
                const KeyT kk = (KeyT(c) << (3 * b)) | (KeyT(cd[c]) << (2 * b)) | (KeyT(cd[gs_slow_class(c)]) << b) | KeyT(cd[gs_fast_class(c)]);
                key[p] = kk;
                int64_t lo = s_first;
                if (i >= first_end) {
                    ++lo;
                    while (lo + 1 < S && off[lo + 1] <= i) ++lo;
                }
                smp = lo;
                ins = (unsigned long long)(kk);
                if (lo - s_first < 8192) fold = (unsigned long long)(lo - s_first) << 50;
                else solo = true;
            }
        }
        const uint32_t peers = __match_any_sync(0xffffffffu, solo ? (0xffffull << 48 | (unsigned long long)(threadIdx.x)) : (ins | fold));
        if (ins != ~0ull && (solo || lane == __ffs(peers) - 1)) {
            bool fresh = true;
            if (!solo) {
                const unsigned long long want = (ins | fold) + 1ull;
                uint32_t h = uint32_t((want * 0x9E3779B97F4A7C15ull) >> 54);
                for (int probe = 0; probe < 16; ++probe) {
                    const unsigned long long cur = atomicCAS(s_seen + h, 0ull, want);
                    if (cur == 0ull) break;
                    if (cur == want) { fresh = false; break; }
                    h = (h + 1u) & uint32_t(SC_SLOTS - 1);
                }
            }
            if (fresh) gh_insert(hash + size_t(smp) * GH_SLOTS, ins, overflow + smp);
        }
    }
}

__global__ void __launch_bounds__(256) k_tile_ranges(const int32_t *__restrict__ mstart, const int32_t *__restrict__ tile_sample,
                                                     const int32_t *__restrict__ tile_first, int32_t n_tiles, int2 *__restrict__ range) {
    const int t = blockIdx.x * blockDim.x + threadIdx.x;
    if (t >= n_tiles) return;
    const int s = tile_sample[t];
    const int lt = t - tile_first[s];
    const int b0 = mstart[s], b1 = mstart[s + 1];
    const int begin = min(b1, b0 + lt * RS_TILE);
    range[t] = make_int2(begin, min(b1, begin + RS_TILE));
}


template <typename KeyT>
__global__ void __launch_bounds__(1024) k_group_rank(const unsigned long long *__restrict__ hash, const double *__restrict__ wtable, int32_t code_bits,
                                                     uint16_t *__restrict__ slot_gid, int32_t *__restrict__ ngroups, KeyT *__restrict__ gkeys,
                                                     double4 *__restrict__ gw, int *__restrict__ overflow) {
    __shared__ unsigned long long sm[GH_SLOTS];
    __shared__ int s_warp[33];
    const int s = blockIdx.x;
    const unsigned long long *tab = hash + size_t(s) * GH_SLOTS;
    unsigned long long v[4];
    int cnt = 0;
#pragma unroll
    for (int j = 0; j < 4; ++j) {
        v[j] = tab[4 * threadIdx.x + j];
        cnt += v[j] != 0ull;
    }
    int n;
    int at = block_excl_scan(cnt, &n, s_warp);
    int P = 1;
    while (P < n) P <<= 1;
    for (int j = threadIdx.x; j < P; j += blockDim.x) sm[j] = ~0ull;
    __syncthreads();
#pragma unroll
    for (int j = 0; j < 4; ++j)
        if (v[j] != 0ull) sm[at++] = ((v[j] - 1ull) << 12) | (unsigned long long)(4 * threadIdx.x + j);
    __syncthreads();
    for (int k = 2; k <= P; k <<= 1) {
        for (int j = k >> 1; j > 0; j >>= 1) {
            for (int i = threadIdx.x; i < P; i += blockDim.x) {
                const int x = i ^ j;
                if (x > i) {
                    const unsigned long long a = sm[i], c = sm[x];
                    const bool up = (i & k) == 0;
                    if ((a > c) == up) { sm[i] = c; sm[x] = a; }
                }
            }
            __syncthreads();
        }
    }
    const int ng = min(n, GH_MAX_GROUPS);
    uint16_t *out = slot_gid + size_t(s) * GH_SLOTS;
    for (int p = threadIdx.x; p < n; p += blockDim.x) {
        const unsigned long long e = sm[p];
        out[e & 4095ull] = uint16_t(min(p, GH_MAX_GROUPS - 1));
        if (p < ng) {
            const KeyT key = KeyT(e >> 12);
            gkeys[size_t(s) * GH_MAX_GROUPS + p] = key;
            double4 w;
            w.x = __ldg(wtable + gs_code(key, 0, code_bits));
            w.y = __ldg(wtable + gs_code(key, 1, code_bits));
            w.z = __ldg(wtable + gs_code(key, 2, code_bits));
            w.w = 0.0;
            gw[size_t(s) * GH_MAX_GROUPS + p] = w;
        }
    }
    if (threadIdx.x == 0) {
        ngroups[s] = ng;
        if (n > GH_MAX_GROUPS) overflow[s] = 1;
    }
}

template <typename KeyT>
__global__ void __launch_bounds__(RS_THREADS) k_group_ids(const KeyT *__restrict__ key, const int2 *__restrict__ range,
                                                         const int32_t *__restrict__ tile_sample, const unsigned long long *__restrict__ hash,
                                                         const uint16_t *__restrict__ slot_gid, const int32_t *__restrict__ ngroups,
                                                         uint16_t *__restrict__ gid, uint32_t *__restrict__ tile_hist) {
    __shared__ uint32_t h[GH_MAX_GROUPS];
    const int t = blockIdx.x;
    const int2 rg = range[t];
    const int begin = rg.x, end = rg.y;
    const int s = tile_sample[t];
    const int ng = ngroups[s];
    if (begin >= end) {
        for (int d = threadIdx.x; d < ng; d += RS_THREADS) tile_hist[size_t(t) * GH_MAX_GROUPS + d] = 0u;
        return;
    }
    for (int d = threadIdx.x; d < ng; d += RS_THREADS) h[d] = 0u;
    const int lane = threadIdx.x & 31, warp = threadIdx.x >> 5;
    const unsigned long long *tab = hash + size_t(s) * GH_SLOTS;
    const uint16_t *sg = slot_gid + size_t(s) * GH_SLOTS;
    KeyT k[RS_PER_THREAD];
#pragma unroll
    for (int e = 0; e < RS_PER_THREAD; ++e) {
        const int i = begin + warp * (32 * RS_PER_THREAD) + e * 32 + lane;
        k[e] = i < end ? key[i] : KeyT(0);
    }
    __syncthreads();
#pragma unroll
    for (int e = 0; e < RS_PER_THREAD; ++e) {
        const int i = begin + warp * (32 * RS_PER_THREAD) + e * 32 + lane;
        if (i < end) {
            const uint32_t g = min(uint32_t(__ldg(sg + gh_find(tab, (unsigned long long)(k[e])))), uint32_t(max(ng, 1) - 1));
            gid[i] = uint16_t(g);
            atomicAdd(h + g, 1u);
        }
    }
    __syncthreads();
    uint32_t *out = tile_hist + size_t(t) * GH_MAX_GROUPS;
    for (int d = threadIdx.x; d < ng; d += RS_THREADS) out[d] = h[d];
}

__global__ void __launch_bounds__(1024) k_group_scan(uint32_t *__restrict__ tile_hist, const int32_t *__restrict__ tile_first,
                                                     const int32_t *__restrict__ ngroups, int32_t *__restrict__ goff) {
    __shared__ int s_warp[33];
    const int s = blockIdx.x;
    const int ng = ngroups[s];
    const int t0 = tile_first[s], t1 = tile_first[s + 1];
    constexpr int PITCH = GH_MAX_GROUPS, U = 8;
    uint32_t tot[2] = {0u, 0u};
    const int d0 = 2 * threadIdx.x;
#pragma unroll
    for (int j = 0; j < 2; ++j) {
        if (d0 + j < ng) {
            uint32_t run = 0u;
            for (int t = t0; t < t1; t += U) {
                uint32_t c[U];
#pragma unroll
                for (int u = 0; u < U; ++u) c[u] = t + u < t1 ? tile_hist[size_t(t + u) * PITCH + d0 + j] : 0u;
#pragma unroll
                for (int u = 0; u < U; ++u) {
                    if (t + u < t1) tile_hist[size_t(t + u) * PITCH + d0 + j] = run;
                    run += c[u];
                }
            }
            tot[j] = run;
        }
    }
    int all;
    const int ex = block_excl_scan(int(tot[0] + tot[1]), &all, s_warp);
    int32_t *out = goff + size_t(s) * (GH_MAX_GROUPS + 1);
    if (d0 < ng) out[d0] = ex;
    if (d0 + 1 < ng) out[d0 + 1] = ex + int(tot[0]);
    if (threadIdx.x == 0) out[ng] = all;
}

__global__ void __launch_bounds__(RS_THREADS, 3) k_group_place(const uint16_t *__restrict__ gid_in,
                                                              const int32_t *__restrict__ pair_db_in, const int32_t *__restrict__ pair_s_in,
                                                              int32_t *__restrict__ pair_db_out, int32_t *__restrict__ pair_s_out,
                                                              const int32_t *__restrict__ mstart, const int32_t *__restrict__ tile_sample,
                                                              const int32_t *__restrict__ tile_first, const int2 *__restrict__ range,
                                                              const uint32_t *__restrict__ tile_hist, const int32_t *__restrict__ ngroups,
                                                              const int32_t *__restrict__ goff, unsigned int *__restrict__ work_counter) {
    extern __shared__ uint32_t rs_sm[];
    if (blockIdx.x == 0 && threadIdx.x == 0) *work_counter = 0u;
    constexpr int NW = RS_THREADS / 32;
    constexpr int PITCH = GH_MAX_GROUPS;
    uint16_t *whist = reinterpret_cast<uint16_t *>(rs_sm);
    uint32_t *off = rs_sm + NW * PITCH / 2;
    const int t = blockIdx.x;
    const int2 rg = range[t];
    const int begin = rg.x, end = rg.y;
    const int s = tile_sample[t];
    if (begin >= end) return;
    const int lane = threadIdx.x & 31, warp = threadIdx.x >> 5;
    uint32_t d[RS_PER_THREAD];
    int32_t pdb[RS_PER_THREAD], ps[RS_PER_THREAD];
#pragma unroll
    for (int e = 0; e < RS_PER_THREAD; ++e) {
        const int i = begin + warp * (32 * RS_PER_THREAD) + e * 32 + lane;
        const bool on = i < end;
        d[e] = on ? uint32_t(gid_in[i]) : 0xffffffffu;
        pdb[e] = on ? pair_db_in[i] : 0;
        ps[e] = on && pair_s_out ? pair_s_in[i] : 0;
    }
    const int ng = ngroups[s];
    const int base = mstart[s];
    for (int j = threadIdx.x; j < NW * PITCH / 2; j += RS_THREADS) rs_sm[j] = 0u;
    for (int g = threadIdx.x; g < ng; g += RS_THREADS)
        off[g] = uint32_t(__ldg(goff + size_t(s) * (GH_MAX_GROUPS + 1) + g)) + __ldg(tile_hist + size_t(t) * PITCH + g);
    __syncthreads();
    const uint32_t lt_mask = (1u << lane) - 1u;
    uint16_t *mine_h = whist + size_t(warp) * PITCH;
    uint32_t rank[RS_PER_THREAD];
#pragma unroll
    for (int e = 0; e < RS_PER_THREAD; ++e) {
        const bool on = d[e] != 0xffffffffu;
        const uint32_t peers = __match_any_sync(0xffffffffu, d[e]);
        uint32_t prior = 0u;
        if (on) prior = mine_h[d[e]];
        __syncwarp();
        if (on && lane == __ffs(peers) - 1) mine_h[d[e]] = uint16_t(prior + __popc(peers));
        __syncwarp();
        rank[e] = prior + uint32_t(__popc(peers & lt_mask));
    }
    __syncthreads();
    for (int g = threadIdx.x; g < ng; g += RS_THREADS) {
        uint32_t run = 0u;
#pragma unroll
        for (int w = 0; w < NW; ++w) {
            const uint32_t c = whist[size_t(w) * PITCH + g];
            whist[size_t(w) * PITCH + g] = uint16_t(run);
            run += c;
        }
    }
    __syncthreads();
#pragma unroll
    for (int e = 0; e < RS_PER_THREAD; ++e) {
        if (d[e] != 0xffffffffu) {
            const int o = base + int(off[d[e]]) + int(mine_h[d[e]]) + int(rank[e]);
            pair_db_out[o] = pdb[e];
            if (pair_s_out) pair_s_out[o] = ps[e];
        }
    }
}

constexpr int SEG_CLASSES = 16;
constexpr int SO_LEVELS = 128;
constexpr int SO_BUCKETS = SEG_CLASSES * SO_LEVELS;
__device__ __forceinline__ int seg_cost_class(int cost, int base) {
    const int r = (cost * 16) / max(base, 1);
    const int lim[SEG_CLASSES - 1] = {384, 256, 192, 160, 128, 96, 80, 64, 48, 40, 32, 28, 24, 20, 18};
    int c = 0;
#pragma unroll
    for (int k = 0; k < SEG_CLASSES - 1; ++k) c += r < lim[k] ? 1 : 0;
    return c;
}

constexpr int SEG_COST_BLOCK = 8;
constexpr int SEG_COST_CHANGE = 8;
template <typename KeyT>
__device__ __forceinline__ void group_marks_body(int s, const int32_t *s_off, int ng, const KeyT *__restrict__ gkeys,
                                                 const int32_t *__restrict__ mstart, const int32_t *__restrict__ seg_off, int32_t chunk,
                                                 int32_t code_bits, unsigned long long *__restrict__ blk_chg, int32_t *__restrict__ seg_cost,
                                                 int32_t jcap, int32_t *__restrict__ bucket_cnt, int2 *__restrict__ seg_br) {
    const int m = mstart[s + 1] - mstart[s];
    const int seg0 = seg_off[s];
    const int nseg_s = seg_off[s + 1] - seg0;
    for (int j = threadIdx.x; j < nseg_s; j += blockDim.x) {
        const int rows = min(chunk, m - j * chunk);
        atomicAdd(seg_cost + seg0 + j, SEG_COST_BLOCK * ((rows + 15) / 16));
    }
    if (m > 0 && ng > 0) {
        unsigned long long *out = blk_chg + size_t(seg0) * size_t(chunk / 16);
        const KeyT *gk = gkeys + size_t(s) * GH_MAX_GROUPS;
        const int b = code_bits;
        for (int g = 1 + threadIdx.x; g < ng; g += blockDim.x) {
            const int r = s_off[g];
            if (r >= m || s_off[g + 1] == r) continue;
            const KeyT k1 = gk[g], k0 = gk[g - 1];
            const int c1 = int(k1 >> (3 * b)) & 3, c0 = int(k0 >> (3 * b)) & 3;
            unsigned long long bits = 0ull;
            if (c1 != c0) {
                bits = 1ull | (1ull << 16) | (1ull << 32);
            } else {
                const KeyT dd = k1 ^ k0;
                const uint32_t fm = (1u << b) - 1u;
#pragma unroll
                for (int w = 0; w < 3; ++w)
                    if ((uint32_t(dd >> gs_field_shift(c1, w, b)) & fm) != 0u) bits |= 1ull << (16 * w);
            }
            atomicOr(out + (r >> 4), bits << (r & 15));
            atomicAdd(seg_cost + seg0 + r / chunk, SEG_COST_CHANGE * __popcll(bits));
        }
        const int nb = (m + 15) / 16;
        for (int blk = threadIdx.x; blk < nb; blk += blockDim.x) {
            int lo = 0, hi = ng;
            const int r = 16 * blk;
            while (hi - lo > 1) {
                const int mid = (lo + hi) >> 1;
                if (s_off[mid] <= r) lo = mid; else hi = mid;
            }
            atomicOr(out + blk, (unsigned long long)(lo) << 48);
        }
    }
    __threadfence();
    __syncthreads();
    const int base = SEG_COST_BLOCK * (chunk / 16);
    const int jdiv = (jcap + SO_LEVELS - 1) / SO_LEVELS;
    for (int j = threadIdx.x; j < nseg_s; j += blockDim.x) {
        const int bkt = seg_cost_class(__ldcg(seg_cost + seg0 + j), base) * SO_LEVELS + min(SO_LEVELS - 1, j / jdiv);
        seg_br[seg0 + j] = make_int2(bkt, atomicAdd(bucket_cnt + bkt, 1));
    }
}

template <typename KeyT>
__global__ void __launch_bounds__(1024) k_group_marks(const int32_t *__restrict__ goff, const KeyT *__restrict__ gkeys, const int32_t *__restrict__ ngroups,
                                                      const int32_t *__restrict__ mstart, const int32_t *__restrict__ seg_off, int32_t chunk,
                                                      int32_t code_bits, unsigned long long *__restrict__ blk_chg, int32_t *__restrict__ seg_cost,
                                                      int32_t jcap, int32_t *__restrict__ bucket_cnt, int2 *__restrict__ seg_br) {
    __shared__ int32_t s_off[GH_MAX_GROUPS + 1];
    const int s = blockIdx.x;
    const int ng = ngroups[s];
    for (int g = threadIdx.x; g <= ng; g += blockDim.x) s_off[g] = goff[size_t(s) * (GH_MAX_GROUPS + 1) + g];
    __syncthreads();
    group_marks_body<KeyT>(s, s_off, ng, gkeys, mstart, seg_off, chunk, code_bits, blk_chg, seg_cost, jcap, bucket_cnt, seg_br);
}

constexpr int GP_WARPS = 32;
constexpr int GP_MAX_PAIRS = 65535;
constexpr size_t GP_SMEM = size_t(GP_WARPS) * GH_MAX_GROUPS * 2 + size_t(GH_MAX_GROUPS + 4) * 4;
template <typename KeyT>
__global__ void __launch_bounds__(32 * GP_WARPS) k_group_sample(
        const KeyT *__restrict__ key, const unsigned long long *__restrict__ hash, const uint16_t *__restrict__ slot_gid,
        const int32_t *__restrict__ ngroups, uint16_t *__restrict__ gid, const int32_t *__restrict__ pair_db_in,
        const int32_t *__restrict__ pair_s_in, int32_t *__restrict__ pair_db_out, int32_t *__restrict__ pair_s_out,
        int32_t *__restrict__ goff, const KeyT *__restrict__ gkeys, const int32_t *__restrict__ mstart,
        const int32_t *__restrict__ seg_off, int32_t chunk, int32_t code_bits, unsigned long long *__restrict__ blk_chg,
        int32_t *__restrict__ seg_cost, int32_t jcap, int32_t *__restrict__ bucket_cnt, int2 *__restrict__ seg_br,
        unsigned int *__restrict__ work_counter) {
    extern __shared__ __align__(16) unsigned char gp_smem[];
    __shared__ int s_warp[33];
    uint16_t *whist = reinterpret_cast<uint16_t *>(gp_smem);
    uint32_t *whist32 = reinterpret_cast<uint32_t *>(gp_smem);
    int32_t *s_off = reinterpret_cast<int32_t *>(gp_smem + size_t(GP_WARPS) * GH_MAX_GROUPS * 2);
    if (blockIdx.x == 0 && threadIdx.x == 0) *work_counter = 0u;
    const int s = blockIdx.x;
    const int ng = ngroups[s];
    const int b0 = mstart[s], m = min(mstart[s + 1] - b0, GP_MAX_PAIRS);
    const int lane = threadIdx.x & 31, warp = threadIdx.x >> 5;
    const int used_words = (ng + 1) / 2;
    for (int j = threadIdx.x; j < GP_WARPS * used_words; j += blockDim.x) whist32[size_t(j / used_words) * (GH_MAX_GROUPS / 2) + j % used_words] = 0u;
    __syncthreads();
    const int per = ((m + GP_WARPS - 1) / GP_WARPS + 31) & ~31;
    const int r0 = min(m, warp * per), r1 = min(m, r0 + per);
    uint16_t *mine = whist + size_t(warp) * GH_MAX_GROUPS;
    const unsigned long long *tab = hash + size_t(s) * GH_SLOTS;
    const uint16_t *sg = slot_gid + size_t(s) * GH_SLOTS;
    const uint32_t last_id = uint32_t(max(ng, 1) - 1);
    constexpr int U = 8;
    for (int base = r0; base < r1; base += 32 * U) {
        unsigned long long want[U], cur[U];
        uint32_t h[U];
#pragma unroll
        for (int u = 0; u < U; ++u) {
            const int i = base + 32 * u + lane;
            want[u] = i < r1 ? (unsigned long long)(key[b0 + i]) + 1ull : 0ull;
            h[u] = gh_hash(want[u] - 1ull);
        }
#pragma unroll
        for (int u = 0; u < U; ++u) cur[u] = want[u] ? __ldg(tab + h[u]) : 0ull;
#pragma unroll
        for (int u = 0; u < U; ++u) {
            for (int probe = 1; probe < GH_SLOTS && cur[u] != want[u] && cur[u] != 0ull; ++probe) {
                h[u] = (h[u] + 1u) & uint32_t(GH_SLOTS - 1);
                cur[u] = __ldg(tab + h[u]);
            }
        }
        uint32_t g[U];
#pragma unroll
        for (int u = 0; u < U; ++u) g[u] = want[u] ? min(uint32_t(__ldg(sg + h[u])), last_id) : 0xffffffffu;
#pragma unroll
        for (int u = 0; u < U; ++u) {
            if (base + 32 * u >= r1) break;
            const int i = base + 32 * u + lane;
            const bool on = i < r1;
            if (on) gid[b0 + i] = uint16_t(g[u]);
            const uint32_t peers = __match_any_sync(0xffffffffu, g[u]);
            if (on && lane == __ffs(peers) - 1) mine[g[u]] = uint16_t(mine[g[u]] + __popc(peers));
            __syncwarp();
        }
    }
    __syncthreads();
    uint32_t tot0 = 0u, tot1 = 0u;
    if (2 * int(threadIdx.x) < ng) {
#pragma unroll 8
        for (int w = 0; w < GP_WARPS; ++w) {
            const uint32_t c = whist32[size_t(w) * (GH_MAX_GROUPS / 2) + threadIdx.x];
            whist32[size_t(w) * (GH_MAX_GROUPS / 2) + threadIdx.x] = tot0 | (tot1 << 16);
            tot0 += c & 0xffffu;
            tot1 += c >> 16;
        }
    }
    int all;
    const int ex = block_excl_scan(int(tot0 + tot1), &all, s_warp);
    int32_t *out = goff + size_t(s) * (GH_MAX_GROUPS + 1);
    const int d0 = 2 * int(threadIdx.x);
    if (d0 < ng) { s_off[d0] = ex; out[d0] = ex; }
    if (d0 + 1 < ng) { s_off[d0 + 1] = ex + int(tot0); out[d0 + 1] = ex + int(tot0); }
    if (threadIdx.x == 0) { s_off[ng] = all; out[ng] = all; }
    __syncthreads();
    const uint32_t lt_mask = (1u << lane) - 1u;
    for (int base = r0; base < r1; base += 32 * U) {
        uint32_t g[U];
        int32_t pdb[U], ps[U];
#pragma unroll
        for (int u = 0; u < U; ++u) {
            const int i = base + 32 * u + lane;
            const bool on = i < r1;
            g[u] = on ? uint32_t(gid[b0 + i]) : 0xffffffffu;
            pdb[u] = on ? pair_db_in[b0 + i] : 0;
            ps[u] = on && pair_s_out ? pair_s_in[b0 + i] : 0;
        }
#pragma unroll
        for (int u = 0; u < U; ++u) {
            if (base + 32 * u >= r1) break;
            const bool on = g[u] != 0xffffffffu;
            const uint32_t peers = __match_any_sync(0xffffffffu, g[u]);
            uint32_t prior = 0u;
            if (on) prior = mine[g[u]];
            __syncwarp();
            if (on && lane == __ffs(peers) - 1) mine[g[u]] = uint16_t(prior + __popc(peers));
            __syncwarp();
            if (on) {
                const int o = b0 + s_off[g[u]] + int(prior) + __popc(peers & lt_mask);
                pair_db_out[o] = pdb[u];
                if (pair_s_out) pair_s_out[o] = ps[u];
            }
        }
    }
    __syncthreads();
    group_marks_body<KeyT>(s, s_off, ng, gkeys, mstart, seg_off, chunk, code_bits, blk_chg, seg_cost, jcap, bucket_cnt, seg_br);
}

__global__ void __launch_bounds__(256) k_order_place(const int32_t *__restrict__ bucket_cnt, const int2 *__restrict__ seg_br, const int32_t *__restrict__ seg_off,
                                                    const int32_t *__restrict__ mstart, int32_t chunk, int4 *__restrict__ order) {
    __shared__ int scan[SO_BUCKETS];
    __shared__ int warp_sum[8];
    const int s = blockIdx.x, t = threadIdx.x;
    const int seg0 = seg_off[s], nseg_s = seg_off[s + 1] - seg0;
    if (nseg_s <= 0) return;
    constexpr int PT = SO_BUCKETS / 256;
    int v[PT], sum = 0;
#pragma unroll
    for (int k = 0; k < PT; ++k) { v[k] = __ldcg(bucket_cnt + PT * t + k); sum += v[k]; }
    int incl = sum;
#pragma unroll
    for (int d = 1; d < 32; d <<= 1) {
        const int u = __shfl_up_sync(0xffffffffu, incl, d);
        if ((t & 31) >= d) incl += u;
    }
    if ((t & 31) == 31) warp_sum[t >> 5] = incl;
    __syncthreads();
    int run = incl - sum;
    for (int w = 0; w < (t >> 5); ++w) run += warp_sum[w];
#pragma unroll
    for (int k = 0; k < PT; ++k) { scan[PT * t + k] = run; run += v[k]; }
    __syncthreads();
    const int m0 = mstart[s], m1 = mstart[s + 1];
    for (int j = t; j < nseg_s; j += blockDim.x) {
        const int2 br = seg_br[seg0 + j];
        const int begin = m0 + j * chunk;
        order[scan[br.x] + br.y] = make_int4(seg0 + j, begin, min(m1, begin + chunk) - begin, s);
    }
}

}
```

Before: 6243 billion.

## Record hash slots at insert time instead of storing keys and re-probing

```diff
diff --git a/snpmatch_b200/csrc/api.cu b/snpmatch_b200/csrc/api.cu
--- a/snpmatch_b200/csrc/api.cu
+++ b/snpmatch_b200/csrc/api.cu
@@ -884,6 +884,15 @@
         for (int64_t t = 0; t < ceil_div64(ns, RS_TILE); ++t) tile_sample.push_back(int32_t(s));
     }
     tile_first[size_t(n_samples)] = int32_t(tile_sample.size());
+    const int64_t n_jt = ceil_div64(n, JOIN_TILE);
+    std::vector<int32_t> join_tiles(size_t(n_jt) * 4);
+    for (int64_t t = 0, s = 0; t < n_jt; ++t) {
+        const int64_t i0 = t * JOIN_TILE, i1 = std::min(n, i0 + JOIN_TILE);
+        while (s + 1 < n_samples && offsets[s + 1] <= i0) ++s;
+        join_tiles[size_t(4 * t)] = int32_t(s);
+        join_tiles[size_t(4 * t + 1)] = int32_t(offsets[s + 1]);
+        join_tiles[size_t(4 * t + 2)] = offsets[s] == i0 || offsets[s + 1] < i1;
+    }
     b->nseg_cap = nseg;
     b->n_sort_tiles = int64_t(tile_sample.size());
     const size_t key_bytes = b->key_bits <= 32 ? 4 : 8;
@@ -893,16 +902,19 @@
     SNPM_TRY(b->d_wei_idx.ensure(size_t(n) * 4));
     SNPM_TRY(b->d_codes.ensure(size_t(n) * 6));
     SNPM_TRY(b->d_wtable.ensure(size_t(n_wtable) * 8));
-    SNPM_TRY(b->d_key_a.ensure(size_t(n) * key_bytes));
+    SNPM_TRY(b->d_pair_slot.ensure(size_t(n) * 2));
     SNPM_TRY(b->d_pair_db_tmp.ensure(size_t(n) * 4));
     SNPM_TRY(b->d_pair_s_tmp.ensure(size_t(n) * 4));
     SNPM_TRY(b->d_tile_sample.ensure(std::max<size_t>(tile_sample.size(), 1) * 4));
     SNPM_TRY(b->d_tile_first.ensure(size_t(n_samples + 1) * 4));
+    SNPM_TRY(b->d_join_tiles.ensure(std::max<size_t>(join_tiles.size(), 4) * 4));
     SNPM_TRY(b->d_tile_hist.ensure(std::max<size_t>(tile_sample.size(), 1) * (size_t(GH_MAX_GROUPS) * 4 + 8)));
     SNPM_TRY(b->d_blk_chg.ensure(size_t(std::max<int64_t>(nseg, 1)) * (size_t(b->gchunk / GR_BLOCK) * 8 + 12) + size_t(SO_BUCKETS) * 4 + 16));
     SNPM_TRY(b->d_seg_order.ensure(size_t(std::max<int64_t>(nseg, 1)) * 16));
     SNPM_TRY(b->d_work_counter.ensure(256));
+    const size_t hash_cap = b->d_hash.cap;
     SNPM_TRY(b->d_hash.ensure(size_t(n_samples) * GH_SLOTS * 8));
+    if (b->d_hash.cap != hash_cap) b->hash_dirty = true;
     SNPM_TRY(b->d_slot_gid.ensure(size_t(n_samples) * GH_SLOTS * 2));
     SNPM_TRY(b->d_ngroups.ensure(size_t(n_samples) * 4));
     SNPM_TRY(b->d_group_overflow.ensure(size_t(n_samples) * 4));
@@ -915,11 +927,15 @@
     b->h_gtable.assign(wtable, wtable + n_wtable);
     b->h_tiles.assign(tile_first.begin(), tile_first.end());
     b->h_tiles.insert(b->h_tiles.end(), tile_sample.begin(), tile_sample.end());
+    b->h_tiles.insert(b->h_tiles.end(), join_tiles.begin(), join_tiles.end());
     SNPM_CUDA(cudaMemcpyAsync(b->d_off.p, offsets, size_t(n_samples + 1) * 8, cudaMemcpyHostToDevice, st));
     SNPM_CUDA(cudaMemcpyAsync(b->d_wtable.p, b->h_gtable.data(), size_t(n_wtable) * 8, cudaMemcpyHostToDevice, st));
     SNPM_CUDA(cudaMemcpyAsync(b->d_tile_first.p, b->h_tiles.data(), size_t(n_samples + 1) * 4, cudaMemcpyHostToDevice, st));
     if (!tile_sample.empty())
         SNPM_CUDA(cudaMemcpyAsync(b->d_tile_sample.p, b->h_tiles.data() + n_samples + 1, tile_sample.size() * 4, cudaMemcpyHostToDevice, st));
+    if (!join_tiles.empty())
+        SNPM_CUDA(cudaMemcpyAsync(b->d_join_tiles.p, b->h_tiles.data() + n_samples + 1 + tile_sample.size(), join_tiles.size() * 4,
+                                  cudaMemcpyHostToDevice, st));
     if (n) {
         SNPM_CUDA(cudaMemcpyAsync(b->d_wei_idx.p, chrom_pos, size_t(n) * 4, cudaMemcpyHostToDevice, st));
         if (codes32) SNPM_CUDA(cudaMemcpyAsync(b->d_codes.p, codes32, size_t(n) * 4, cudaMemcpyHostToDevice, st));
@@ -1037,8 +1053,8 @@
                       &b->d_win_count, &b->d_win_off, &b->d_win_begin, &b->d_win_end, &b->d_kmax, &b->d_win_L, &b->d_win_LR,
                       &b->d_win_ident, &b->d_win_amb, &b->d_win_row_off, &b->d_row_acc, &b->d_row_score, &b->d_row_ninfo, &b->d_row_L, &b->d_row_ident, &b->d_f1_acc, &b->d_f1_part, &b->d_f1_out, &b->d_pair_code, &b->d_wei_idx, &b->d_wei_table,
                       &b->d_chrom8, &b->d_gid, &b->d_gtable, &b->d_pair_gid, &b->d_part_int, &b->d_guard, &b->d_runs,
-                      &b->d_codes, &b->d_wtable, &b->d_key_a, &b->d_key_b, &b->d_idx_a, &b->d_idx_b, &b->d_pair_db_tmp, &b->d_pair_s_tmp,
-                      &b->d_tile_sample, &b->d_tile_first, &b->d_tile_hist, &b->d_blk_chg, &b->d_seg_order, &b->d_work_counter, &b->d_hash, &b->d_slot_gid, &b->d_ngroups,
+                      &b->d_codes, &b->d_wtable, &b->d_pair_slot, &b->d_pair_db_tmp, &b->d_pair_s_tmp,
+                      &b->d_tile_sample, &b->d_tile_first, &b->d_join_tiles, &b->d_tile_hist, &b->d_blk_chg, &b->d_seg_order, &b->d_work_counter, &b->d_hash, &b->d_slot_gid, &b->d_ngroups,
                       &b->d_group_overflow, &b->d_gkeys, &b->d_gw, &b->d_goff, &b->d_segsel, &b->d_segsel_off, &b->d_flags, &b->d_flag_counts};
     for (DevBuf *d : bufs) d->release();
     for (int i = 0; i < SNPM_N_EVENTS; ++i)
@@ -1188,17 +1204,19 @@
         SNPM_KERNEL_CHECK();
         if (b->coded) {
             unsigned long long *hash = b->d_hash.as<unsigned long long>();
-            SNPM_CUDA(cudaMemsetAsync(hash, 0, size_t(S) * GH_SLOTS * 8, st));
+            if (b->hash_dirty) SNPM_CUDA(cudaMemsetAsync(hash, 0, b->d_hash.cap, st));
+            int32_t *pair_s = b->track_pairs ? b->d_pair_s_tmp.as<int32_t>() : nullptr;
             if (b->key_bits <= 32)
                 k_scatter_pairs_coded<uint32_t><<<int(n_tiles), SC_THREADS, 0, st>>>(b->d_match_row.as<int32_t>(), n, b->d_tile_off.as<int32_t>(), b->d_codes.as<uint16_t>(),
-                        b->d_wtable.as<double>(), b->n_wtable, b->code_bits, b->d_prefix.as<int32_t>(), b->d_pair_db_tmp.as<int32_t>(), b->d_pair_s_tmp.as<int32_t>(),
-                        b->d_key_a.as<uint32_t>(), b->d_status.as<int>(), b->d_off.as<int64_t>(), S, hash, b->d_group_overflow.as<int>(),
-                        b->codes_packed ? b->d_codes.as<uint32_t>() : nullptr);
+                        b->d_wtable.as<double>(), b->n_wtable, b->code_bits, b->d_prefix.as<int32_t>(), b->d_pair_db_tmp.as<int32_t>(), pair_s,
+                        b->d_pair_slot.as<uint16_t>(), b->d_status.as<int>(), b->d_off.as<int64_t>(), b->d_join_tiles.as<int4>(), S, hash,
+                        b->d_group_overflow.as<int>(), b->codes_packed ? b->d_codes.as<uint32_t>() : nullptr);
             else
                 k_scatter_pairs_coded<uint64_t><<<int(n_tiles), SC_THREADS, 0, st>>>(b->d_match_row.as<int32_t>(), n, b->d_tile_off.as<int32_t>(), b->d_codes.as<uint16_t>(),
-                        b->d_wtable.as<double>(), b->n_wtable, b->code_bits, b->d_prefix.as<int32_t>(), b->d_pair_db_tmp.as<int32_t>(), b->d_pair_s_tmp.as<int32_t>(),
-                        b->d_key_a.as<uint64_t>(), b->d_status.as<int>(), b->d_off.as<int64_t>(), S, hash, b->d_group_overflow.as<int>(),
-                        b->codes_packed ? b->d_codes.as<uint32_t>() : nullptr);
+                        b->d_wtable.as<double>(), b->n_wtable, b->code_bits, b->d_prefix.as<int32_t>(), b->d_pair_db_tmp.as<int32_t>(), pair_s,
+                        b->d_pair_slot.as<uint16_t>(), b->d_status.as<int>(), b->d_off.as<int64_t>(), b->d_join_tiles.as<int4>(), S, hash,
+                        b->d_group_overflow.as<int>(), b->codes_packed ? b->d_codes.as<uint32_t>() : nullptr);
+            b->hash_dirty = true;
         } else if (b->grouped)
             k_scatter_pairs_grouped<<<int(n_tiles), JOIN_TILE, 0, st>>>(b->d_match_row.as<int32_t>(), n, b->d_tile_off.as<int32_t>(),
                                                                       b->d_gid.as<uint16_t>(), b->n_gtable, b->d_prefix.as<int32_t>(), b->d_pair_db.as<int32_t>(),
@@ -1234,6 +1252,8 @@
     KeyT *gkeys = b->d_gkeys.as<KeyT>();
     k_group_rank<KeyT><<<int(b->S), 1024, 0, st>>>(b->d_hash.as<unsigned long long>(), b->d_wtable.as<double>(), b->code_bits, b->d_slot_gid.as<uint16_t>(),
                                                    b->d_ngroups.as<int32_t>(), gkeys, b->d_gw.as<double4>(), b->d_group_overflow.as<int>());
+    SNPM_KERNEL_CHECK();
+    b->hash_dirty = false;
     int64_t n_max = 0, jcap1 = 1;
     for (int64_t s = 0; s < b->S; ++s) {
         n_max = std::max(n_max, b->h_off[size_t(s) + 1] - b->h_off[size_t(s)]);
@@ -1251,7 +1271,7 @@
         int2 *br = reinterpret_cast<int2 *>(reinterpret_cast<unsigned char *>(b->d_blk_chg.p) + ((zbytes + 7) & ~size_t(7)));
         SNPM_CUDA(cudaMemsetAsync(b->d_blk_chg.p, 0, zbytes, st));
         k_group_sample<KeyT><<<int(b->S), 32 * GP_WARPS, GP_SMEM, st>>>(
-            b->d_key_a.as<KeyT>(), b->d_hash.as<unsigned long long>(), b->d_slot_gid.as<uint16_t>(), b->d_ngroups.as<int32_t>(), b->d_gid.as<uint16_t>(),
+            b->d_pair_slot.as<uint16_t>(), b->d_slot_gid.as<uint16_t>(), b->d_ngroups.as<int32_t>(), b->d_gid.as<uint16_t>(),
             b->d_pair_db_tmp.as<int32_t>(), b->d_pair_s_tmp.as<int32_t>(), b->d_pair_db.as<int32_t>(), b->track_pairs ? b->d_pair_s.as<int32_t>() : nullptr,
             b->d_goff.as<int32_t>(), gkeys, mstart, b->d_seg_off.as<int32_t>(), b->gchunk, b->code_bits, b->d_blk_chg.as<unsigned long long>(), cost,
             int32_t(jcap1), buckets, br, b->d_work_counter.as<unsigned int>());
@@ -1261,8 +1281,8 @@
         return SNPM_OK;
     }
     k_tile_ranges<<<(tiles + 255) / 256, 256, 0, st>>>(mstart, tsample, tfirst, tiles, range);
-    k_group_ids<KeyT><<<tiles, RS_THREADS, 0, st>>>(b->d_key_a.as<KeyT>(), range, tsample, b->d_hash.as<unsigned long long>(), b->d_slot_gid.as<uint16_t>(),
-                                                    b->d_ngroups.as<int32_t>(), b->d_gid.as<uint16_t>(), hist);
+    k_group_ids<<<tiles, RS_THREADS, 0, st>>>(b->d_pair_slot.as<uint16_t>(), range, tsample, b->d_slot_gid.as<uint16_t>(), b->d_ngroups.as<int32_t>(),
+                                              b->d_gid.as<uint16_t>(), hist);
     k_group_scan<<<int(b->S), 1024, 0, st>>>(hist, tfirst, b->d_ngroups.as<int32_t>(), b->d_goff.as<int32_t>());
     const size_t nseg_cap = size_t(std::max<int64_t>(b->nseg_cap, 1));
     int32_t *seg_cost = reinterpret_cast<int32_t *>(b->d_blk_chg.as<unsigned long long>() + nseg_cap * size_t(b->gchunk / GR_BLOCK));
diff --git a/snpmatch_b200/csrc/common.cuh b/snpmatch_b200/csrc/common.cuh
--- a/snpmatch_b200/csrc/common.cuh
+++ b/snpmatch_b200/csrc/common.cuh
@@ -144,8 +144,9 @@
     bool codes_packed = false;
     int32_t n_wtable = 0, code_bits = 0, key_bits = 0;
     int64_t n_sort_tiles = 0;
-    snpm::DevBuf d_codes, d_wtable, d_key_a, d_key_b, d_idx_a, d_idx_b, d_pair_db_tmp, d_pair_s_tmp, d_tile_sample, d_tile_first,
+    snpm::DevBuf d_codes, d_wtable, d_pair_slot, d_pair_db_tmp, d_pair_s_tmp, d_tile_sample, d_tile_first, d_join_tiles,
                  d_tile_hist, d_blk_chg, d_seg_order, d_work_counter, d_hash, d_slot_gid, d_ngroups, d_group_overflow, d_gkeys, d_gw, d_goff;
+    bool hash_dirty = true;
     bool track_pairs = true;
     cudaEvent_t ev_fork = nullptr, ev_join = nullptr;
     cudaEvent_t ev_joined = nullptr;
diff --git a/snpmatch_b200/csrc/group_sort.cuh b/snpmatch_b200/csrc/group_sort.cuh
--- a/snpmatch_b200/csrc/group_sort.cuh
+++ b/snpmatch_b200/csrc/group_sort.cuh
@@ -23,25 +23,16 @@
 constexpr int GH_MAX_GROUPS = 2048;
 
 __device__ __forceinline__ uint32_t gh_hash(unsigned long long key) { return uint32_t((key * 0x9E3779B97F4A7C15ull) >> 52); }
-__device__ __forceinline__ void gh_insert(unsigned long long *__restrict__ table, unsigned long long key, int *overflow) {
+__device__ __forceinline__ uint32_t gh_insert(unsigned long long *__restrict__ table, unsigned long long key, int *overflow) {
     const unsigned long long want = key + 1ull;
     uint32_t h = gh_hash(key);
     for (int probe = 0; probe < GH_SLOTS; ++probe) {
         unsigned long long cur = __ldcg(table + h);
         if (cur == 0ull) cur = atomicCAS(table + h, 0ull, want);
-        if (cur == 0ull || cur == want) return;
+        if (cur == 0ull || cur == want) return h;
         h = (h + 1u) & uint32_t(GH_SLOTS - 1);
     }
     atomicExch(overflow, 1);
-}
-__device__ __forceinline__ uint32_t gh_find(const unsigned long long *__restrict__ table, unsigned long long key) {
-    const unsigned long long want = key + 1ull;
-    uint32_t h = gh_hash(key);
-    for (int probe = 0; probe < GH_SLOTS; ++probe) {
-        const unsigned long long cur = __ldg(table + h);
-        if (cur == want || cur == 0ull) break;
-        h = (h + 1u) & uint32_t(GH_SLOTS - 1);
-    }
     return h;
 }
 
@@ -49,16 +40,17 @@
 constexpr int SC_PER = JOIN_TILE / SC_THREADS;
 constexpr int SC_SLOTS = 1024;
 template <typename KeyT>
-__global__ void __launch_bounds__(SC_THREADS) k_scatter_pairs_coded(
+__global__ void __launch_bounds__(SC_THREADS, 6) k_scatter_pairs_coded(
         const int32_t *__restrict__ match_row, int64_t n, const int32_t *__restrict__ tile_off, const uint16_t *__restrict__ codes,
         const double *__restrict__ wtable, int32_t n_table, int32_t code_bits, int32_t *__restrict__ prefix,
-        int32_t *__restrict__ pair_db, int32_t *__restrict__ pair_s, KeyT *__restrict__ key, int *status,
-        const int64_t *__restrict__ off, int64_t S, unsigned long long *__restrict__ hash, int *__restrict__ overflow,
-        const uint32_t *__restrict__ codes32) {
+        int32_t *__restrict__ pair_db, int32_t *__restrict__ pair_s, uint16_t *__restrict__ pair_slot, int *status,
+        const int64_t *__restrict__ off, const int4 *__restrict__ join_tiles, int64_t S, unsigned long long *__restrict__ hash,
+        int *__restrict__ overflow, const uint32_t *__restrict__ codes32) {
     constexpr int NW = SC_THREADS / 32;
-    __shared__ int s_cnt[SC_PER][NW];
-    __shared__ int64_t s_first_sm, s_first_end;
+    constexpr uint32_t SEEN = 1u << 12;
+    __shared__ uint32_t s_bal[SC_PER][NW];
     __shared__ unsigned long long s_seen[SC_SLOTS];
+    __shared__ uint16_t s_slot[SC_SLOTS];
     const int lane = threadIdx.x & 31, warp = threadIdx.x >> 5;
     const int64_t i0 = int64_t(blockIdx.x) * JOIN_TILE;
     int32_t row[SC_PER];
@@ -74,91 +66,114 @@
         cw[j] = (codes32 != nullptr && i < n) ? codes32[i] : 0u;
     }
     const int32_t base0 = tile_off[blockIdx.x];
+    const int4 tm = __ldg(join_tiles + blockIdx.x);
 #pragma unroll
     for (int j = 0; j < SC_SLOTS / SC_THREADS; ++j) s_seen[j * SC_THREADS + threadIdx.x] = 0ull;
     uint32_t bal[SC_PER];
 #pragma unroll
     for (int j = 0; j < SC_PER; ++j) {
         bal[j] = __ballot_sync(0xffffffffu, row[j] >= 0);
-        if (lane == 0) s_cnt[j][warp] = __popc(bal[j]);
-    }
-    if (threadIdx.x == 0) {
-        int64_t lo = 0, hi = S;
-        while (hi - lo > 1) {
+        if (lane == 0) s_bal[j][warp] = bal[j];
+    }
+    __syncthreads();
+    if (tm.z && warp == NW - 1) {
+        const int64_t i1 = min(n, i0 + JOIN_TILE);
+        const uint32_t *bf = &s_bal[0][0];
+        int64_t lo = 0, hi = int64_t(tm.x) + 1;
+        while (lo < hi) {
             const int64_t mid = (lo + hi) >> 1;
-            if (off[mid] <= i0) lo = mid; else hi = mid;
-        }
-        s_first_sm = lo;
-        s_first_end = off[lo + 1];
-    }
-    __syncthreads();
-    const int64_t s_first = s_first_sm, first_end = s_first_end;
+            if (off[mid] < i0) lo = mid + 1; else hi = mid;
+        }
+        for (int64_t s = lo + lane; s < S; s += 32) {
+            const int64_t o = off[s];
+            if (o >= i1) break;
+            const int r = int(o - i0);
+            int32_t v = base0 + __popc(bf[r >> 5] & ((1u << (r & 31)) - 1u));
+            for (int k = 0; k < (r >> 5); ++k) v += __popc(bf[k]);
+            prefix[o] = v;
+        }
+    }
+    const int64_t s_first = tm.x, first_end = tm.y;
     int32_t base = base0;
+    int32_t pp[SC_PER];
+    uint32_t link[SC_PER];
 #pragma unroll
     for (int j = 0; j < SC_PER; ++j) {
         const int64_t i = i0 + j * SC_THREADS + threadIdx.x;
         int before = 0, total = 0;
 #pragma unroll
         for (int w = 0; w < NW; ++w) {
-            const int c = s_cnt[j][w];
+            const int c = __popc(s_bal[j][w]);
             before += w < warp ? c : 0;
             total += c;
         }
         const int32_t p = base + before + __popc(bal[j] & ((1u << lane) - 1u));
         base += total;
+        pp[j] = -1;
         unsigned long long ins = ~0ull, fold = 0ull;
         bool solo = false;
         int64_t smp = 0;
-        if (i < n) {
-            prefix[i] = p;
-            if (row[j] >= 0) {
-                pair_db[p] = row[j];
-                pair_s[p] = int32_t(i);
-                uint32_t cd[3];
-                if (codes32 != nullptr) {
-                    const uint32_t v = cw[j];
-                    cd[0] = v & 1023u; cd[2] = (v >> 10) & 1023u; cd[1] = (v >> 20) & 1023u;
-                } else {
-                    cd[0] = codes[3 * i]; cd[2] = codes[3 * i + 1]; cd[1] = codes[3 * i + 2];
-                }
-                bool bad = false;
-#pragma unroll
-                for (int k = 0; k < 3; ++k)
-                    if (int32_t(cd[k]) >= n_table) { bad = true; cd[k] = 0; }
-                if (bad) atomicAdd(status + 4, 1);
-                const double w0 = __ldg(wtable + cd[0]), w1 = __ldg(wtable + cd[1]), w2 = __ldg(wtable + cd[2]);
-                int c;
-                if (w0 == 1.0) c = 0; else if (w1 == 1.0) c = 1; else if (w2 == 1.0) c = 2;
-                else { c = 0; if (w1 > w0) c = 1; if (w2 > (c ? w1 : w0)) c = 2; }
-                const int b = code_bits;
-                const KeyT kk = (KeyT(c) << (3 * b)) | (KeyT(cd[c]) << (2 * b)) | (KeyT(cd[gs_slow_class(c)]) << b) | KeyT(cd[gs_fast_class(c)]);
-                key[p] = kk;
-                int64_t lo = s_first;
-                if (i >= first_end) {
-                    ++lo;
-                    while (lo + 1 < S && off[lo + 1] <= i) ++lo;
-                }
-                smp = lo;
-                ins = (unsigned long long)(kk);
-                if (lo - s_first < 8192) fold = (unsigned long long)(lo - s_first) << 50;
-                else solo = true;
-            }
+        if (i < n && row[j] >= 0) {
+            pp[j] = p;
+            pair_db[p] = row[j];
+            if (pair_s != nullptr) pair_s[p] = int32_t(i);
+            uint32_t cd[3];
+            if (codes32 != nullptr) {
+                const uint32_t v = cw[j];
+                cd[0] = v & 1023u; cd[2] = (v >> 10) & 1023u; cd[1] = (v >> 20) & 1023u;
+            } else {
+                cd[0] = codes[3 * i]; cd[2] = codes[3 * i + 1]; cd[1] = codes[3 * i + 2];
+            }
+            bool bad = false;
+#pragma unroll
+            for (int k = 0; k < 3; ++k)
+                if (int32_t(cd[k]) >= n_table) { bad = true; cd[k] = 0; }
+            if (bad) atomicAdd(status + 4, 1);
+            const double w0 = __ldg(wtable + cd[0]), w1 = __ldg(wtable + cd[1]), w2 = __ldg(wtable + cd[2]);
+            int c;
+            if (w0 == 1.0) c = 0; else if (w1 == 1.0) c = 1; else if (w2 == 1.0) c = 2;
+            else { c = 0; if (w1 > w0) c = 1; if (w2 > (c ? w1 : w0)) c = 2; }
+            const int b = code_bits;
+            const KeyT kk = (KeyT(c) << (3 * b)) | (KeyT(cd[c]) << (2 * b)) | (KeyT(cd[gs_slow_class(c)]) << b) | KeyT(cd[gs_fast_class(c)]);
+            int64_t lo = s_first;
+            if (i >= first_end) {
+                ++lo;
+                while (lo + 1 < S && off[lo + 1] <= i) ++lo;
+            }
+            smp = lo;
+            ins = (unsigned long long)(kk);
+            if (lo - s_first < 8192) fold = (unsigned long long)(lo - s_first) << 50;
+            else solo = true;
         }
         const uint32_t peers = __match_any_sync(0xffffffffu, solo ? (0xffffull << 48 | (unsigned long long)(threadIdx.x)) : (ins | fold));
-        if (ins != ~0ull && (solo || lane == __ffs(peers) - 1)) {
+        const int leader = __ffs(peers) - 1;
+        link[j] = uint32_t(leader) << 16;
+        if (ins != ~0ull && lane == leader) {
             bool fresh = true;
+            int entry = -1;
             if (!solo) {
                 const unsigned long long want = (ins | fold) + 1ull;
                 uint32_t h = uint32_t((want * 0x9E3779B97F4A7C15ull) >> 54);
                 for (int probe = 0; probe < 16; ++probe) {
                     const unsigned long long cur = atomicCAS(s_seen + h, 0ull, want);
-                    if (cur == 0ull) break;
-                    if (cur == want) { fresh = false; break; }
+                    if (cur == 0ull) { entry = int(h); break; }
+                    if (cur == want) { fresh = false; link[j] |= SEEN | h; break; }
                     h = (h + 1u) & uint32_t(SC_SLOTS - 1);
                 }
             }
-            if (fresh) gh_insert(hash + size_t(smp) * GH_SLOTS, ins, overflow + smp);
-        }
+            if (fresh) {
+                const uint32_t slot = gh_insert(hash + size_t(smp) * GH_SLOTS, ins, overflow + smp);
+                if (entry >= 0) s_slot[entry] = uint16_t(slot);
+                link[j] |= slot;
+            }
+        }
+    }
+    __syncthreads();
+#pragma unroll
+    for (int j = 0; j < SC_PER; ++j) {
+        const uint32_t v = (link[j] & SEEN) ? uint32_t(s_slot[link[j] & (SC_SLOTS - 1)]) : (link[j] & (GH_SLOTS - 1));
+        const uint32_t slot = __shfl_sync(0xffffffffu, v, int(link[j] >> 16));
+        if (pp[j] >= 0) pair_slot[pp[j]] = uint16_t(slot);
     }
 }
 
@@ -175,13 +190,13 @@
 
 
 template <typename KeyT>
-__global__ void __launch_bounds__(1024) k_group_rank(const unsigned long long *__restrict__ hash, const double *__restrict__ wtable, int32_t code_bits,
+__global__ void __launch_bounds__(1024) k_group_rank(unsigned long long *__restrict__ hash, const double *__restrict__ wtable, int32_t code_bits,
                                                      uint16_t *__restrict__ slot_gid, int32_t *__restrict__ ngroups, KeyT *__restrict__ gkeys,
                                                      double4 *__restrict__ gw, int *__restrict__ overflow) {
     __shared__ unsigned long long sm[GH_SLOTS];
     __shared__ int s_warp[33];
     const int s = blockIdx.x;
-    const unsigned long long *tab = hash + size_t(s) * GH_SLOTS;
+    unsigned long long *tab = hash + size_t(s) * GH_SLOTS;
     unsigned long long v[4];
     int cnt = 0;
 #pragma unroll
@@ -189,6 +204,8 @@
         v[j] = tab[4 * threadIdx.x + j];
         cnt += v[j] != 0ull;
     }
+#pragma unroll
+    for (int j = 0; j < 4; ++j) tab[4 * threadIdx.x + j] = 0ull;
     int n;
     int at = block_excl_scan(cnt, &n, s_warp);
     int P = 1;
@@ -199,17 +216,40 @@
     for (int j = 0; j < 4; ++j)
         if (v[j] != 0ull) sm[at++] = ((v[j] - 1ull) << 12) | (unsigned long long)(4 * threadIdx.x + j);
     __syncthreads();
-    for (int k = 2; k <= P; k <<= 1) {
-        for (int j = k >> 1; j > 0; j >>= 1) {
-            for (int i = threadIdx.x; i < P; i += blockDim.x) {
-                const int x = i ^ j;
-                if (x > i) {
-                    const unsigned long long a = sm[i], c = sm[x];
-                    const bool up = (i & k) == 0;
-                    if ((a > c) == up) { sm[i] = c; sm[x] = a; }
+    if (n <= 1024) {
+        const int i = threadIdx.x;
+        unsigned long long a = i < n ? sm[i] : ~0ull;
+        int buf = 1;
+        for (int k = 2; k <= P; k <<= 1) {
+            for (int j = k >> 1; j > 0; j >>= 1) {
+                unsigned long long c;
+                if (j < 32) {
+                    c = __shfl_xor_sync(0xffffffffu, a, j);
+                } else {
+                    sm[GH_SLOTS / 2 * buf + i] = a;
+                    __syncthreads();
+                    c = sm[GH_SLOTS / 2 * buf + (i ^ j)];
+                    buf ^= 1;
                 }
-            }
-            __syncthreads();
+                a = (((i & j) == 0) == ((i & k) == 0)) ? min(a, c) : max(a, c);
+            }
+        }
+        __syncthreads();
+        sm[i] = a;
+        __syncthreads();
+    } else {
+        for (int k = 2; k <= P; k <<= 1) {
+            for (int j = k >> 1; j > 0; j >>= 1) {
+                for (int i = threadIdx.x; i < P; i += blockDim.x) {
+                    const int x = i ^ j;
+                    if (x > i) {
+                        const unsigned long long a = sm[i], c = sm[x];
+                        const bool up = (i & k) == 0;
+                        if ((a > c) == up) { sm[i] = c; sm[x] = a; }
+                    }
+                }
+                __syncthreads();
+            }
         }
     }
     const int ng = min(n, GH_MAX_GROUPS);
@@ -234,11 +274,10 @@
     }
 }
 
-template <typename KeyT>
-__global__ void __launch_bounds__(RS_THREADS) k_group_ids(const KeyT *__restrict__ key, const int2 *__restrict__ range,
-                                                         const int32_t *__restrict__ tile_sample, const unsigned long long *__restrict__ hash,
-                                                         const uint16_t *__restrict__ slot_gid, const int32_t *__restrict__ ngroups,
-                                                         uint16_t *__restrict__ gid, uint32_t *__restrict__ tile_hist) {
+__global__ void __launch_bounds__(RS_THREADS) k_group_ids(const uint16_t *__restrict__ pair_slot, const int2 *__restrict__ range,
+                                                         const int32_t *__restrict__ tile_sample, const uint16_t *__restrict__ slot_gid,
+                                                         const int32_t *__restrict__ ngroups, uint16_t *__restrict__ gid,
+                                                         uint32_t *__restrict__ tile_hist) {
     __shared__ uint32_t h[GH_MAX_GROUPS];
     const int t = blockIdx.x;
     const int2 rg = range[t];
@@ -251,20 +290,19 @@
     }
     for (int d = threadIdx.x; d < ng; d += RS_THREADS) h[d] = 0u;
     const int lane = threadIdx.x & 31, warp = threadIdx.x >> 5;
-    const unsigned long long *tab = hash + size_t(s) * GH_SLOTS;
     const uint16_t *sg = slot_gid + size_t(s) * GH_SLOTS;
-    KeyT k[RS_PER_THREAD];
+    uint32_t sl[RS_PER_THREAD];
 #pragma unroll
     for (int e = 0; e < RS_PER_THREAD; ++e) {
         const int i = begin + warp * (32 * RS_PER_THREAD) + e * 32 + lane;
-        k[e] = i < end ? key[i] : KeyT(0);
+        sl[e] = i < end ? uint32_t(pair_slot[i]) : 0u;
     }
     __syncthreads();
 #pragma unroll
     for (int e = 0; e < RS_PER_THREAD; ++e) {
         const int i = begin + warp * (32 * RS_PER_THREAD) + e * 32 + lane;
         if (i < end) {
-            const uint32_t g = min(uint32_t(__ldg(sg + gh_find(tab, (unsigned long long)(k[e])))), uint32_t(max(ng, 1) - 1));
+            const uint32_t g = min(uint32_t(__ldg(sg + sl[e])), uint32_t(max(ng, 1) - 1));
             gid[i] = uint16_t(g);
             atomicAdd(h + g, 1u);
         }
@@ -465,7 +503,7 @@
 constexpr size_t GP_SMEM = size_t(GP_WARPS) * GH_MAX_GROUPS * 2 + size_t(GH_MAX_GROUPS + 4) * 4;
 template <typename KeyT>
 __global__ void __launch_bounds__(32 * GP_WARPS) k_group_sample(
-        const KeyT *__restrict__ key, const unsigned long long *__restrict__ hash, const uint16_t *__restrict__ slot_gid,
+        const uint16_t *__restrict__ pair_slot, const uint16_t *__restrict__ slot_gid,
         const int32_t *__restrict__ ngroups, uint16_t *__restrict__ gid, const int32_t *__restrict__ pair_db_in,
         const int32_t *__restrict__ pair_s_in, int32_t *__restrict__ pair_db_out, int32_t *__restrict__ pair_s_out,
         int32_t *__restrict__ goff, const KeyT *__restrict__ gkeys, const int32_t *__restrict__ mstart,
@@ -488,31 +526,19 @@
     const int per = ((m + GP_WARPS - 1) / GP_WARPS + 31) & ~31;
     const int r0 = min(m, warp * per), r1 = min(m, r0 + per);
     uint16_t *mine = whist + size_t(warp) * GH_MAX_GROUPS;
-    const unsigned long long *tab = hash + size_t(s) * GH_SLOTS;
     const uint16_t *sg = slot_gid + size_t(s) * GH_SLOTS;
     const uint32_t last_id = uint32_t(max(ng, 1) - 1);
     constexpr int U = 8;
     for (int base = r0; base < r1; base += 32 * U) {
-        unsigned long long want[U], cur[U];
-        uint32_t h[U];
+        uint32_t sl[U];
 #pragma unroll
         for (int u = 0; u < U; ++u) {
             const int i = base + 32 * u + lane;
-            want[u] = i < r1 ? (unsigned long long)(key[b0 + i]) + 1ull : 0ull;
-            h[u] = gh_hash(want[u] - 1ull);
-        }
-#pragma unroll
-        for (int u = 0; u < U; ++u) cur[u] = want[u] ? __ldg(tab + h[u]) : 0ull;
-#pragma unroll
-        for (int u = 0; u < U; ++u) {
-            for (int probe = 1; probe < GH_SLOTS && cur[u] != want[u] && cur[u] != 0ull; ++probe) {
-                h[u] = (h[u] + 1u) & uint32_t(GH_SLOTS - 1);
-                cur[u] = __ldg(tab + h[u]);
-            }
+            sl[u] = i < r1 ? uint32_t(pair_slot[b0 + i]) : 0xffffffffu;
         }
         uint32_t g[U];
 #pragma unroll
-        for (int u = 0; u < U; ++u) g[u] = want[u] ? min(uint32_t(__ldg(sg + h[u])), last_id) : 0xffffffffu;
+        for (int u = 0; u < U; ++u) g[u] = sl[u] != 0xffffffffu ? min(uint32_t(__ldg(sg + sl[u])), last_id) : 0xffffffffu;
 #pragma unroll
         for (int u = 0; u < U; ++u) {
             if (base + 32 * u >= r1) break;
```

New measurement: 6388 billion, median of 6. +2.3%, better.
